# aicell-lab/bioengine-worker

Measured on AMD Instinct MI355X. Metric: cellpose_cyto3_512x512_imgs_per_sec, higher is better.
Workload: dtype bf16; 1 GPU; model=cellpose-cyto3 CPnet (nbase 2-32-64-128-256, style on, BN folded), global_batch=32, parallelism=dp1 (replica per GPU)

## Files before the change

### bioengine_worker_amd/ops/conv_pair.py

```python
from __future__ import annotations

from dataclasses import dataclass

import torch
import torch.nn.functional as F

from . import _native
from .conv import INMODES, PackedConv, _act_ref, _affine_stride, fused_conv2d, fused_conv2d_ref, out_hw

SUPPORTED = {
    (8, 32, "none", False, True, "none"),
    (32, 32, "none", False, False, "full"),
    (64, 32, "up2", True, False, "up2"),
    (32, 64, "pool2", False, False, "full"),
    (64, 64, "none", False, False, "full"),
    (128, 64, "up2", True, False, "up2"),
}
RESMODES = {"none": 0, "full": 1, "up2": 2}
FRAG_CONFIGS = {
    (64, 64, "none", False, False, "full"),
    (32, 64, "pool2", False, False, "full"),
    (128, 64, "up2", True, False, "up2"),
}
PROJ_CONFIGS = {
    (32, 64, "pool2", False, True, "none"),
}
SUPPORTED |= PROJ_CONFIGS


def pack_proj_frag(wp: torch.Tensor) -> torch.Tensor:
    cout, nchunk, kp = wp.shape
    assert cout == 64 and nchunk == 1 and kp == 32, "projection fragments: 32 -> 64 channels, 1x1"
    t = wp.reshape(4, 16, 4, 8)
    return t.permute(0, 2, 1, 3).contiguous().reshape(1, 4, 64, 8)


def unpack_proj_frag(wf: torch.Tensor) -> torch.Tensor:
    return wf.reshape(4, 4, 16, 8).permute(0, 2, 1, 3).contiguous().reshape(64, 1, 32)


def pack_frag(wp: torch.Tensor) -> torch.Tensor:
    cout, nchunk, kp = wp.shape
    assert cout == 64 and kp == 288, "fragment packing: 64 output channels, 3x3 taps of 32-channel chunks"
    t = wp.reshape(4, 16, nchunk, 9, 4, 8)
    return t.permute(2, 3, 0, 4, 1, 5).contiguous().reshape(nchunk, 9, 4, 64, 8)


def unpack_frag(wf: torch.Tensor) -> torch.Tensor:
    nchunk = wf.shape[0]
    t = wf.reshape(nchunk, 9, 4, 4, 16, 8)
    return t.permute(2, 4, 0, 1, 3, 5).contiguous().reshape(64, nchunk, 288)


@dataclass
class PairSpec:

    pa: PackedConv
    pb: PackedConv
    sa: torch.Tensor
    ta: torch.Tensor | None
    sb: torch.Tensor
    tb: torch.Tensor | None
    bias: torch.Tensor
    inmode: str = "none"
    pp: PackedConv | None = None
    sp: torch.Tensor | None = None
    tp: torch.Tensor | None = None
    frag_cache: dict | None = None
    bias_p: torch.Tensor | None = None
    proj_frag_cache: dict | None = None
    plain: "PairSpec | None" = None

    def proj_rounded(self, has_x2: bool, res: str) -> bool:
        return self.bias_p is not None and (self.cin, self.cm, self.inmode, has_x2, self.pp is not None, res) in PROJ_CONFIGS

    def frag_proj(self, device: torch.device) -> torch.Tensor:
        key = (str(device), self.pp.wp.data_ptr())
        if self.proj_frag_cache is None or self.proj_frag_cache.get("key") != key:
            self.proj_frag_cache = {"key": key, "w": pack_proj_frag(self.pp.wp.to(device))}
        return self.proj_frag_cache["w"]

    def frag(self, device: torch.device) -> tuple[torch.Tensor, torch.Tensor]:
        key = (str(device), self.pa.wp.data_ptr(), self.pb.wp.data_ptr())
        if self.frag_cache is None:
            self.frag_cache = {}
        if self.frag_cache.get("key") != key:
            self.frag_cache.update(key=key, w=(pack_frag(self.pa.wp.to(device)), pack_frag(self.pb.wp.to(device))))
        return self.frag_cache["w"]

    @property
    def cm(self) -> int:
        return self.pb.cout

    @property
    def cin(self) -> int:
        return self.pa.cin_pad

    def supports(self, has_x2: bool, res: str) -> bool:
        cfg = (self.cin, self.cm, self.inmode, has_x2, self.pp is not None, res)
        return cfg in SUPPORTED and (cfg in PROJ_CONFIGS) == (self.bias_p is not None)

    def without_proj(self) -> "PairSpec":
        if self.frag_cache is None:
            self.frag_cache = {}
        if self.plain is None:
            self.plain = PairSpec(pa=self.pa, pb=self.pb, sa=self.sa, ta=self.ta, sb=self.sb, tb=self.tb,
                                  bias=self.bias, inmode=self.inmode, frag_cache=self.frag_cache)
        return self.plain


def fold_bias(shift: torch.Tensor, scale: torch.Tensor, bias: torch.Tensor | None) -> torch.Tensor:
    if bias is None:
        return shift.clone()
    n = bias.numel()
    out = shift.clone()
    out[..., :n] = out[..., :n] + scale[:n] * bias.to(shift.device)
    return out


def conv_pair_ref(x, spec: PairSpec, *, ta=None, tb=None, x2=None, res=None, res_mode="none"):
    ta = spec.ta if ta is None else ta
    tb = spec.tb if tb is None else tb
    if spec.proj_rounded(x2 is not None, "none" if res is None else res_mode):
        proj = fused_conv2d_ref(x, spec.pp, scale=spec.sp, shift=spec.tp, inmode=spec.inmode)
        return conv_pair_ref(x, spec.without_proj(), ta=ta, tb=tb, res=proj, res_mode="full")
    xf = x.float()
    a = _act_ref(xf, None, spec.sa, ta, True, spec.inmode).to(torch.bfloat16).float()
    wa = spec.pa.w.to(a.device)
    if wa.shape[1] < a.shape[1]:
        wa = F.pad(wa, (0, 0, 0, 0, 0, a.shape[1] - wa.shape[1]))
    hA = F.conv2d(a, wa.to(torch.bfloat16).float(), None, padding=1)
    if x2 is not None:
        hA = hA + x2.float().permute(0, 3, 1, 2)
    C = hA.shape[1]
    sb = spec.sb[:C].view(1, C, 1, 1)
    tbv = tb.view(-1, tb.shape[-1], 1, 1)[:, :C] if tb.dim() == 2 else tb[:C].view(1, C, 1, 1)
    h = torch.relu(hA * sb + tbv).to(torch.bfloat16).float()
    y = F.conv2d(h, spec.pb.w.to(h.device).to(torch.bfloat16).float(), None, padding=1)
    if spec.pp is not None:
        p = _act_ref(xf, None, spec.sp, spec.tp, False, spec.inmode).to(torch.bfloat16).float()
        wp = spec.pp.w.to(p.device)
        if wp.shape[1] < p.shape[1]:
            wp = F.pad(wp, (0, 0, 0, 0, 0, p.shape[1] - wp.shape[1]))
        y = y + F.conv2d(p, wp.to(torch.bfloat16).float(), None)
    y = y + spec.bias.to(y.device).view(1, -1, 1, 1)
    y = y.permute(0, 2, 3, 1)
    if res is not None:
        r = res.float()
        if res_mode == "up2":
            r = r.repeat_interleave(2, 1).repeat_interleave(2, 2)
        y = y + r
    return y.to(x.dtype).contiguous()


def conv_pair(x: torch.Tensor, spec: PairSpec, *, ta=None, tb=None, x2=None, res=None, res_mode: str = "none",
              out: torch.Tensor | None = None) -> torch.Tensor:
    ta = spec.ta if ta is None else ta
    tb = spec.tb if tb is None else tb
    assert ta is not None and tb is not None, "conv_pair needs actA / actB shifts"
    if res is None:
        res_mode = "none"
    if not x.is_cuda:
        y = conv_pair_ref(x, spec, ta=ta, tb=tb, x2=x2, res=res, res_mode=res_mode)
        if out is not None:
            out.copy_(y)
            return out
        return y
    N, Hs, Ws, Cin = x.shape
    H, W = out_hw(x, spec.inmode)
    CM = spec.cm
    assert x.dtype == torch.bfloat16 and x.is_contiguous(), "conv_pair expects contiguous NHWC bf16"
    assert Cin == spec.cin, f"input channels {Cin} != packed {spec.cin}"
    if spec.proj_rounded(x2 is not None, res_mode):
        return _conv_pair_proj(x, spec, ta, tb, out)
    if not spec.supports(x2 is not None, res_mode):
        raise ValueError(f"conv_pair: unsupported configuration {(Cin, CM, spec.inmode, x2 is not None, spec.pp is not None, res_mode)}")
    if x2 is not None:
        assert x2.shape == (N, H, W, CM) and x2.dtype == torch.bfloat16 and x2.is_contiguous()
    if res_mode == "full":
        assert res.shape == (N, H, W, CM) and res.dtype == torch.bfloat16 and res.is_contiguous()
    elif res_mode == "up2":
        assert res.shape == (N, H // 2, W // 2, CM) and res.dtype == torch.bfloat16 and res.is_contiguous()
    if out is None:
        out = torch.empty(N, H, W, CM, device=x.device, dtype=torch.bfloat16)
    else:
        assert out.shape == (N, H, W, CM) and out.dtype == torch.bfloat16 and out.is_contiguous()
        assert out.data_ptr() != x.data_ptr(), "conv_pair cannot run in place"
    ta_ns = _affine_stride(ta, N, Cin)
    tb_ns = _affine_stride(tb, N, CM)
    pp = spec.pp
    waf = wbf = None
    if (Cin, CM, spec.inmode, x2 is not None, pp is not None, res_mode) in FRAG_CONFIGS:
        waf, wbf = spec.frag(x.device)
    _native.call(
        "be_conv_pair_frag",
        _native.ptr(x), _native.ptr(x2), _native.ptr(spec.sa), _native.ptr(ta), ta_ns, _native.ptr(spec.sb),
        _native.ptr(tb), tb_ns, _native.ptr(spec.sp), _native.ptr(spec.tp), _native.ptr(spec.pa.wp),
        _native.ptr(spec.pb.wp), _native.ptr(None if pp is None else pp.wp), _native.ptr(spec.bias),
        _native.ptr(res), _native.ptr(out), N, H, W, Hs, Ws, Cin, CM, INMODES[spec.inmode], int(pp is not None),
        RESMODES[res_mode], _native.ptr(waf), _native.ptr(wbf), _native.stream(x.device),
    )
    return out


def proj_fused(x: torch.Tensor, spec: PairSpec) -> bool:
    H, W = out_hw(x, spec.inmode)
    return x.is_cuda and bool(_native.hip().be_conv_pair_proj_takes(x.shape[0], H, W))


def _conv_pair_proj(x, spec: PairSpec, ta, tb, out):
    N, Hs, Ws, Cin = x.shape
    H, W = out_hw(x, spec.inmode)
    if not proj_fused(x, spec):
        proj = fused_conv2d(x, spec.pp, scale=spec.sp, shift=spec.tp, inmode=spec.inmode)
        return conv_pair(x, spec.without_proj(), ta=ta, tb=tb, res=proj, res_mode="full", out=out)
    CM = spec.cm
    if out is None:
        out = torch.empty(N, H, W, CM, device=x.device, dtype=torch.bfloat16)
    else:
        assert out.shape == (N, H, W, CM) and out.dtype == torch.bfloat16 and out.is_contiguous()
        assert out.data_ptr() != x.data_ptr(), "conv_pair cannot run in place"
    waf, wbf = spec.frag(x.device)
    _native.call(
        "be_conv_pair_proj",
        _native.ptr(x), _native.ptr(spec.sa), _native.ptr(ta), _affine_stride(ta, N, Cin), _native.ptr(spec.sb),
        _native.ptr(tb), _affine_stride(tb, N, CM), _native.ptr(spec.sp), _native.ptr(spec.tp), _native.ptr(spec.pa.wp),
        _native.ptr(spec.pb.wp), _native.ptr(spec.bias), _native.ptr(spec.bias_p), _native.ptr(out), N, H, W, Hs, Ws,
        Cin, CM, _native.ptr(waf), _native.ptr(wbf), _native.ptr(spec.frag_proj(x.device)), _native.stream(x.device),
    )
    return out


@dataclass
class HeadSpec:

    s: torch.Tensor
    t: torch.Tensor
    w: torch.Tensor
    b: torch.Tensor
    nh: int
    wh: torch.Tensor | None = None

    @staticmethod
    def k_order() -> list[int]:
        return [(kq * 4 + j) if j < 4 else (16 + kq * 4 + j - 4) for kq in range(4) for j in range(8)]

    @classmethod
    def build(cls, scale: torch.Tensor, shift: torch.Tensor, weight: torch.Tensor, bias: torch.Tensor | None):
        nh, cin = weight.shape[0], weight.shape[1]
        assert cin <= 32 and nh <= 16 and weight.shape[2:] == (1, 1)
        dev = weight.device
        w = torch.zeros(nh, 32, device=dev)
        w[:, :cin] = weight.detach().float().reshape(nh, cin)
        b = torch.zeros(16, device=dev)
        if bias is not None:
            b[:nh] = bias.detach().float()
        s = torch.zeros(32, device=dev)
        t = torch.zeros(32, device=dev)
        s[: scale.numel()] = scale.float()
        t[: shift.numel()] = shift.float()
        wp = torch.zeros(16, 32, device=dev)
        wp[:nh] = w[:, cls.k_order()]
        return cls(s=s.contiguous(), t=t.contiguous(), w=w, b=b.contiguous(), nh=nh,
                   wh=wp.to(torch.bfloat16).contiguous())


def head_ref(xout: torch.Tensor, head: HeadSpec) -> torch.Tensor:
    a = torch.relu(xout.float() * head.s.to(xout.device) + head.t.to(xout.device))
    w = head.w.to(a.device)
    if xout.dtype == torch.bfloat16:
        a = a.to(torch.bfloat16).float()
        w = w.to(torch.bfloat16).float()
    y = torch.einsum("nhwc,oc->nohw", a, w) + head.b[: head.nh].to(a.device).view(1, -1, 1, 1)
    return y.contiguous()


def conv_pair_head(x: torch.Tensor, spec: PairSpec, head: HeadSpec, *, ta=None, tb=None, res=None) -> torch.Tensor:
    ta = spec.ta if ta is None else ta
    tb = spec.tb if tb is None else tb
    assert ta is not None and tb is not None and res is not None
    if not x.is_cuda:
        return head_ref(conv_pair_ref(x, spec, ta=ta, tb=tb, res=res, res_mode="full"), head)
    N, H, W, Cin = x.shape
    assert spec.cin == 32 and spec.cm == 32 and spec.inmode == "none" and spec.pp is None, "head fusion: 32->32 only"
    assert x.dtype == torch.bfloat16 and x.is_contiguous() and Cin == 32
    assert res.shape == (N, H, W, 32) and res.dtype == torch.bfloat16 and res.is_contiguous()
    hout = torch.empty(N, head.nh, H, W, device=x.device, dtype=torch.float32)
    _native.call(
        "be_conv_pair_head",
        _native.ptr(x), _native.ptr(spec.sa), _native.ptr(ta), _affine_stride(ta, N, Cin), _native.ptr(spec.sb),
        _native.ptr(tb), _affine_stride(tb, N, 32), _native.ptr(spec.pa.wp), _native.ptr(spec.pb.wp),
        _native.ptr(spec.bias), _native.ptr(res), _native.ptr(head.s), _native.ptr(head.t), _native.ptr(head.wh),
        _native.ptr(head.b), _native.ptr(hout), head.nh, N, H, W, _native.stream(x.device),
    )
    return hout
```

### csrc/kernels/common.h

```cpp
#pragma once
#include <hip/hip_runtime.h>
#include <stdint.h>
#include <cstdio>
#include <cstdlib>

typedef uint16_t bf16_t;
typedef __attribute__((ext_vector_type(8))) short bf16x8;
typedef __attribute__((ext_vector_type(4))) float f32x4;
typedef __attribute__((ext_vector_type(4))) uint32_t u32x4;
typedef __attribute__((ext_vector_type(2))) uint32_t u32x2;

#define BE_WAVE 64

__device__ __forceinline__ float bf2f(uint16_t v) { return __uint_as_float(((uint32_t)v) << 16); }

typedef __attribute__((ext_vector_type(2))) float f32x2_t;
typedef __attribute__((ext_vector_type(2))) __bf16 bf16x2_t;

__device__ __forceinline__ uint16_t f2bf(float f) { return __builtin_bit_cast(uint16_t, (__bf16)f); }

__device__ __forceinline__ uint32_t pack2bf(float lo, float hi) {
  const f32x2_t v = {lo, hi};
  return __builtin_bit_cast(uint32_t, __builtin_convertvector(v, bf16x2_t));
}

typedef __attribute__((ext_vector_type(2))) short s16x2_t;
__device__ __forceinline__ uint32_t relu_bf16x2(uint32_t w) {
  const s16x2_t z = {0, 0};
  return __builtin_bit_cast(uint32_t, __builtin_elementwise_max(__builtin_bit_cast(s16x2_t, w), z));
}

__device__ __forceinline__ float lo_bf(uint32_t w) { return __uint_as_float(w << 16); }
__device__ __forceinline__ float hi_bf(uint32_t w) { return __uint_as_float(w & 0xffff0000u); }

__device__ __forceinline__ float wave_sum(float v) {
#pragma unroll
  for (int o = 32; o > 0; o >>= 1) v += __shfl_xor(v, o, 64);
  return v;
}
__device__ __forceinline__ float wave_max(float v) {
#pragma unroll
  for (int o = 32; o > 0; o >>= 1) v = fmaxf(v, __shfl_xor(v, o, 64));
  return v;
}

__device__ __forceinline__ int xcd_remap(int orig, int nwg) {
  const int q = nwg / 8, r = nwg % 8;
  const int xcd = orig % 8;
  const int base = (xcd < r) ? xcd * (q + 1) : r * (q + 1) + (xcd - r) * q;
  return base + orig / 8;
}

#define BE_CHECK_LAUNCH() ((int)hipGetLastError())

inline int be_env_int(const char* name, int dflt) {
  const char* e = getenv(name);
  return e ? atoi(e) : dflt;
}

#define BE_MAX_DEV 64
inline int be_cur_dev() {
  int d = 0;
  (void)hipGetDevice(&d);
  return (d < 0 || d >= BE_MAX_DEV) ? 0 : d;
}

inline const bf16_t* be_zero_page(int slot, size_t bytes) {
  static bf16_t* pages[4][BE_MAX_DEV] = {};
  bf16_t*& z = pages[slot & 3][be_cur_dev()];
  if (!z) {
    if (hipMalloc((void**)&z, bytes) != hipSuccess) { z = nullptr; return nullptr; }
    if (hipMemset(z, 0, bytes) != hipSuccess) return nullptr;
  }
  return z;
}
```

### csrc/kernels/conv_pair.hip

```cpp
#include <cstdlib>

#include "common.h"

namespace {

struct PairArgs {
  const bf16_t* x;
  const bf16_t* x2;
  const float* sa; const float* ta; int ta_ns;
  const float* sb; const float* tb; int tb_ns;
  const float* sp; const float* tp;
  const bf16_t* wa;
  const bf16_t* wb;
  const bf16_t* wp;
  const float* bias;
  const bf16_t* waf; const bf16_t* wbf;
  const bf16_t* wpf; const float* biasp;
  const bf16_t* res;
  bf16_t* out;
  const float* sh; const float* th;
  const bf16_t* wh;
  const float* bh;
  float* hout;
  int nh;
  int N, H, W, Hs, Ws, Cin;
  int tiles_x, tiles_y;
  unsigned long long* stamps;
};

namespace g32 {
constexpr int TW = 32, TH = 16, NW = 8;
#include "conv_pair_onegroup.inc"
}
using namespace g32;

unsigned long long* g_pair_stamps = nullptr;
int g_pair_stamps_cap = 0;

static int g_pair_var = (be_env_int("BE_PAIR_LATE_EPI", 1) ? 1 : 0) | (be_env_int("BE_PAIR_ROLL", 1) ? 2 : 0) |
                        (be_env_int("BE_PAIR_EARLY_AFF", 1) ? 4 : 0) | (be_env_int("BE_PAIR_EPIA", 0) ? 8 : 0) |
                        (be_env_int("BE_PAIR_SEPS", 0) ? 16 : 0) | (be_env_int("BE_PAIR_TOPEPI", 0) ? 32 : 0);

template <int CK, int CM, int INMODE, bool X2, bool PROJ, int RES, int NCA, bool HEAD, bool STAMP, int VAR>
int launch_pair_l(PairArgs a, int g, hipStream_t s) {
  using C = PC<CK, CM, INMODE, X2, PROJ, RES, NCA>;
  constexpr bool seps = (VAR & 16) != 0 && C::RESW && !HEAD;
  constexpr size_t lds = C::LDS + (seps ? (size_t)C::R_OUT * sizeof(bf16_t) : 0);
  static_assert(lds <= 160 * 1024, "LDS budget (separate output staging)");
  static bool attr_set[BE_MAX_DEV] = {};
  if (!attr_set[be_cur_dev()]) {
    hipFuncSetAttribute(
        reinterpret_cast<const void*>(&conv_pair_kernel<CK, CM, INMODE, X2, PROJ, RES, NCA, HEAD, STAMP, VAR>),
        hipFuncAttributeMaxDynamicSharedMemorySize, (int)lds);
    attr_set[be_cur_dev()] = true;
  }
  hipLaunchKernelGGL((conv_pair_kernel<CK, CM, INMODE, X2, PROJ, RES, NCA, HEAD, STAMP, VAR>), dim3(g), dim3(NT), lds, s,
                     a);
  return BE_CHECK_LAUNCH();
}

template <int CK, int CM, int INMODE, bool X2, bool PROJ, int RES, int NCA, bool HEAD = false, bool STAMP = false>
int launch_pair_k(PairArgs a, int g, hipStream_t s) {
  if constexpr (CM == 32 && CK == 32 && !HEAD) {
    if (g_pair_var & 16) {
      if constexpr (NCA == 1)
        if (g_pair_var & 32) return launch_pair_l<CK, CM, INMODE, X2, PROJ, RES, NCA, HEAD, STAMP, 48>(a, g, s);
      return launch_pair_l<CK, CM, INMODE, X2, PROJ, RES, NCA, HEAD, STAMP, 16>(a, g, s);
    }
  }
  if constexpr (CM == 32 && NCA == 1) {
    if (g_pair_var & 32) return launch_pair_l<CK, CM, INMODE, X2, PROJ, RES, NCA, HEAD, STAMP, 32>(a, g, s);
  }
  if constexpr (CM == 64 && RES != 0) {
    switch (g_pair_var & 15) {
      case 1: return launch_pair_l<CK, CM, INMODE, X2, PROJ, RES, NCA, HEAD, STAMP, 1>(a, g, s);
      case 2: return launch_pair_l<CK, CM, INMODE, X2, PROJ, RES, NCA, HEAD, STAMP, 2>(a, g, s);
      case 3: return launch_pair_l<CK, CM, INMODE, X2, PROJ, RES, NCA, HEAD, STAMP, 3>(a, g, s);
      case 5: return launch_pair_l<CK, CM, INMODE, X2, PROJ, RES, NCA, HEAD, STAMP, 5>(a, g, s);
      case 7: return launch_pair_l<CK, CM, INMODE, X2, PROJ, RES, NCA, HEAD, STAMP, 7>(a, g, s);
      case 15: return launch_pair_l<CK, CM, INMODE, X2, PROJ, RES, NCA, HEAD, STAMP, 15>(a, g, s);
      default: break;
    }
  }
  return launch_pair_l<CK, CM, INMODE, X2, PROJ, RES, NCA, HEAD, STAMP, 0>(a, g, s);
}

template <int CK, int CM, int INMODE, bool X2, bool PROJ, int RES, int NCA, bool HEAD = false>
int launch_pair(PairArgs a, int grid_cap, hipStream_t s) {
  a.tiles_x = (a.W + TW - 1) / TW;
  a.tiles_y = (a.H + TH - 1) / TH;
  const int tiles = a.N * a.tiles_x * a.tiles_y;
  int g = grid_cap > 0 ? grid_cap : 256;
  if (g > tiles) g = tiles;
  if (g < 1) return 0;
  a.stamps = nullptr;
  if constexpr (!HEAD && !PROJ && CK == 32) {
    if (g_pair_stamps != nullptr) {
      if (g > g_pair_stamps_cap) return -30;
      a.stamps = g_pair_stamps;
      return launch_pair_k<CK, CM, INMODE, X2, PROJ, RES, NCA, HEAD, true>(a, g, s);
    }
  }
  return launch_pair_k<CK, CM, INMODE, X2, PROJ, RES, NCA, HEAD, false>(a, g, s);
}

#ifndef PP_VAR
#define PP_VAR 1
#endif
#ifndef PP_GW
#define PP_GW 4
#endif
namespace ppk {
constexpr int GW = PP_GW, GT = GW * 64;
constexpr int NTP = 2 * GT;
constexpr int RPW = TH / GW;
constexpr int IN_B = IPIX * 64;
constexpr int H_B = RPIX * 64;
constexpr int OUTW_B = RPW * TW * 64;
constexpr int RB = IN_B;
constexpr int WSTR = 9 * 32 + 16;
constexpr int W_B = 32 * WSTR * 2;
constexpr int APT = 40 / GW, BPT = 32 / GW;
constexpr int TLAST0 = GW * (APT - 1);
constexpr int HU = IPIX * 4;
constexpr int HUPT = (HU + GT - 1) / GT;
static_assert(H_B <= RB && GW * OUTW_B <= RB, "ping-pong region overlays");
static_assert(APT * GW >= RPT && (APT - 1) * GW <= 2 * RH && BPT * GW * 16 == TH * TW, "tile maps");
static_assert(GW == 4 || GW == 8, "group size");
}

struct PPHalo {
  u32x4 h[ppk::HUPT];
  float4 aff[4];
};

__device__ __forceinline__ int pp_in_off(int pi, int c) {
  const int y = pi / IW, x = pi - y * IW;
  return pi * 64 + ((c ^ ((((x >> 2) ^ y) & 1) << 1)) << 4);
}

template <int INMODE, int CIN, bool INT = false>
__device__ __forceinline__ void pp_issue_halo(const PairArgs& a, TileXY t, int ch, int gt, PPHalo& hr) {
  const int c = ch * 32 + (gt & 3) * 8;
  hr.aff[0] = *reinterpret_cast<const float4*>(a.sa + c);
  hr.aff[1] = *reinterpret_cast<const float4*>(a.sa + c + 4);
  const float* tr = a.ta + (size_t)t.n * a.ta_ns + c;
  hr.aff[2] = *reinterpret_cast<const float4*>(tr);
  hr.aff[3] = *reinterpret_cast<const float4*>(tr + 4);
#pragma unroll
  for (int i = 0; i < ppk::HUPT; ++i) {
    const int pi = min(gt + i * ppk::GT, ppk::HU - 1) >> 2;
    const int y = pi / IW, x = pi - y * IW;
    const int gy = INT ? t.ty0 - 2 + y : min(max(t.ty0 - 2 + y, 0), a.H - 1);
    const int gx = INT ? t.tx0 - 2 + x : min(max(t.tx0 - 2 + x, 0), a.W - 1);
    if constexpr (INMODE == 0)
      hr.h[i] = *reinterpret_cast<const u32x4*>(a.x + (((size_t)t.n * a.Hs + gy) * a.Ws + gx) * CIN + c);
    else
      hr.h[i] = *reinterpret_cast<const u32x4*>(a.x + (((size_t)t.n * a.Hs + (gy >> 1)) * a.Ws + (gx >> 1)) * CIN + c);
  }
}

__device__ __forceinline__ bool pp_interior(const PairArgs& a, TileXY t) {
  return t.ty0 >= 2 && t.ty0 + TH + 2 <= a.H && t.tx0 >= 2 && t.tx0 + TW + 2 <= a.W;
}

template <bool INT>
__device__ __forceinline__ void pp_commit(const PairArgs& a, TileXY t, int gt, const PPHalo& hr, unsigned char* rin) {
  float sc[8], sh[8];
  unpack_aff(hr.aff, sc, sh);
  const int c = gt & 3;
#pragma unroll
  for (int i = 0; i < ppk::HUPT; ++i) {
    const int u = gt + i * ppk::GT;
    if (u >= ppk::HU) continue;
    const int pi = u >> 2;
    const int y = pi / IW, x = pi - y * IW;
    const int gy = t.ty0 - 2 + y, gx = t.tx0 - 2 + x;
    u32x4 pk = (u32x4){0u, 0u, 0u, 0u};
    if (INT || (gy >= 0 && gy < a.H && gx >= 0 && gx < a.W)) {
#pragma unroll
      for (int j = 0; j < 4; ++j)
        pk[j] = relu_bf16x2(pack2bf(fmaf(lo_bf(hr.h[i][j]), sc[2 * j], sh[2 * j]),
                                    fmaf(hi_bf(hr.h[i][j]), sc[2 * j + 1], sh[2 * j + 1])));
    }
    *reinterpret_cast<u32x4*>(rin + pi * 64 + ((c ^ ((((x >> 2) ^ y) & 1) << 1)) << 4)) = pk;
  }
}

__device__ __forceinline__ void pp_mma_a(f32x4 (&acc)[2][ppk::APT], const unsigned char* rin, const bf16_t* wa, int gw,
                                         int lrow, int kq) {
  const int par = (gw >> 1) & 1;
  const int b0 = ((gw >> 1) * IW + (gw & 1) * 16 + lrow) * 64;
  int A0[3][2];
#pragma unroll
  for (int dx = 0; dx < 3; ++dx)
#pragma unroll
    for (int pr = 0; pr < 2; ++pr)
      A0[dx][pr] = b0 + dx * 64 + ((kq ^ (((((lrow + dx) >> 2) ^ par ^ pr) & 1) << 1)) << 4);
  int L[3][2];
  const int tl = gw + ppk::TLAST0;
  if (tl < 2 * RH) {
    const int ryl = tl >> 1, rxl = (tl & 1) * 16 + lrow;
#pragma unroll
    for (int dx = 0; dx < 3; ++dx)
#pragma unroll
      for (int pr = 0; pr < 2; ++pr)
        L[dx][pr] = (ryl * IW + rxl + dx) * 64 + ((kq ^ (((((lrow + dx) >> 2) ^ ryl ^ pr) & 1) << 1)) << 4);
  } else {
    int ry9 = (tl - 2 * RH) * 8 + (lrow >> 1), rx9 = 32 + (lrow & 1);
    if (ry9 >= RH) { ry9 = 0; rx9 = 0; }
#pragma unroll
    for (int dx = 0; dx < 3; ++dx)
#pragma unroll
      for (int pr = 0; pr < 2; ++pr)
        L[dx][pr] = (ry9 * IW + rx9 + dx) * 64 + ((kq ^ ((((ry9 & 1) ^ pr) & 1) << 1)) << 4);
  }
  auto frags = [&](int ks, bf16x8 (&af)[2], bf16x8 (&bf)[ppk::APT]) {
    const int dy = ks / 3, dx = ks % 3;
#pragma unroll
    for (int ct = 0; ct < 2; ++ct)
      af[ct] = *reinterpret_cast<const bf16x8*>(wa + (ct * 16 + lrow) * ppk::WSTR + ks * 32 + kq * 8);
#pragma unroll
    for (int j = 0; j < ppk::APT - 1; ++j)
      bf[j] = *reinterpret_cast<const bf16x8*>(rin + A0[dx][dy & 1] + j * (ppk::GW / 2) * IW * 64 + dy * IW * 64);
    bf[ppk::APT - 1] = *reinterpret_cast<const bf16x8*>(rin + L[dx][dy & 1] + dy * IW * 64);
  };
  bf16x8 af[2], afn[2], bf[ppk::APT];
  frags(0, af, bf);
#pragma unroll
  for (int ks = 0; ks < 9; ++ks) {
    const bool more = ks + 1 < 9;
    const int kn = more ? ks + 1 : ks, dy = kn / 3, dx = kn % 3;
#pragma unroll
    for (int j = 0; j < ppk::APT; ++j) {
#pragma unroll
      for (int ct = 0; ct < 2; ++ct) {
        acc[ct][j] = __builtin_amdgcn_mfma_f32_16x16x32_bf16(af[ct], bf[j], acc[ct][j], 0, 0, 0);
        if (j == 0 && more)
          afn[ct] = *reinterpret_cast<const bf16x8*>(wa + (ct * 16 + lrow) * ppk::WSTR + kn * 32 + kq * 8);
      }
      if (more) {
        if (j < ppk::APT - 1)
          bf[j] = *reinterpret_cast<const bf16x8*>(rin + A0[dx][dy & 1] + j * (ppk::GW / 2) * IW * 64 + dy * IW * 64);
        else
          bf[j] = *reinterpret_cast<const bf16x8*>(rin + L[dx][dy & 1] + dy * IW * 64);
      }
      __builtin_amdgcn_sched_barrier(0);
    }
    if (more) {
      af[0] = afn[0];
      af[1] = afn[1];
    }
  }
}

struct PPSkip {
  u32x2 xv[ppk::APT][2];
};

__device__ __forceinline__ bool pp_last(int gw, int lrow, int& ry, int& rx) {
  const int tl = gw + ppk::TLAST0;
  if (tl < 2 * RH) {
    ry = tl >> 1;
    rx = (tl & 1) * 16 + lrow;
    return true;
  }
  ry = (tl - 2 * RH) * 8 + (lrow >> 1);
  rx = 32 + (lrow & 1);
  return ry < RH;
}

__device__ __forceinline__ void pp_issue_skip(const PairArgs& a, TileXY t, int gw, int lrow, int kq, PPSkip& sk) {
#pragma unroll
  for (int j = 0; j < ppk::APT; ++j) {
    int ry, rx;
    if (j < ppk::APT - 1) {
      ry = (gw >> 1) + (ppk::GW / 2) * j;
      rx = (gw & 1) * 16 + lrow;
    } else {
      pp_last(gw, lrow, ry, rx);
    }
    const int gy = min(max(t.ty0 - 1 + ry, 0), a.H - 1), gx = min(max(t.tx0 - 1 + rx, 0), a.W - 1);
    const bf16_t* xp = a.x2 + (((size_t)t.n * a.H + gy) * a.W + gx) * 32 + kq * 4;
#pragma unroll
    for (int ct = 0; ct < 2; ++ct) sk.xv[j][ct] = *reinterpret_cast<const u32x2*>(xp + ct * 16);
  }
}

template <bool X2, bool INT>
__device__ __forceinline__ void pp_epi_a(const PairArgs& a, TileXY t, const f32x4 (&acc)[2][ppk::APT],
                                         unsigned char* rh, const float4 (&s)[2], const float4 (&sh)[2],
                                         const PPSkip& sk, int gw, int lrow, int kq) {
#pragma unroll
  for (int ct = 0; ct < 2; ++ct) {
    const int hc = ((2 * ct) | (kq >> 1));
    const int hw = (((gw >> 1) * RW + (gw & 1) * 16 + lrow) * 64) + ((hc ^ ((lrow >> 1) & 3)) << 4) + (kq & 1) * 8;
#pragma unroll
    for (int j = 0; j < ppk::APT; ++j) {
      int ry, rx, off;
      if (j < ppk::APT - 1) {
        ry = (gw >> 1) + (ppk::GW / 2) * j;
        rx = (gw & 1) * 16 + lrow;
        off = hw + j * (ppk::GW / 2) * RW * 64;
      } else {
        if (!pp_last(gw, lrow, ry, rx)) continue;
        off = (ry * RW + rx) * 64 + ((hc ^ ((rx >> 1) & 3)) << 4) + (kq & 1) * 8;
      }
      const int gy = t.ty0 - 1 + ry, gx = t.tx0 - 1 + rx;
      float v0 = acc[ct][j][0], v1 = acc[ct][j][1], v2 = acc[ct][j][2], v3 = acc[ct][j][3];
      if constexpr (X2) {
        u32x2 xv = sk.xv[j][ct];
        asm volatile("" : "+v"(xv));
        v0 += lo_bf(xv[0]); v1 += hi_bf(xv[0]); v2 += lo_bf(xv[1]); v3 += hi_bf(xv[1]);
      }
      u32x2 st = (u32x2){0u, 0u};
      if (INT || (gy >= 0 && gy < a.H && gx >= 0 && gx < a.W)) {
        st[0] = relu_bf16x2(pack2bf(fmaf(v0, s[ct].x, sh[ct].x), fmaf(v1, s[ct].y, sh[ct].y)));
        st[1] = relu_bf16x2(pack2bf(fmaf(v2, s[ct].z, sh[ct].z), fmaf(v3, s[ct].w, sh[ct].w)));
      }
      *reinterpret_cast<u32x2*>(rh + off) = st;
    }
  }
}

__device__ __forceinline__ void pp_mma_b(f32x4 (&acc)[2][ppk::BPT], const unsigned char* rh, const bf16_t* wb, int gw,
                                         int lrow, int kq) {
  int B0[3];
#pragma unroll
  for (int dx = 0; dx < 3; ++dx) B0[dx] = ((ppk::RPW * gw) * RW + lrow + dx) * 64 + ((kq ^ (((lrow + dx) >> 1) & 3)) << 4);
  auto frags = [&](int ks, bf16x8 (&af)[2], bf16x8 (&bf)[ppk::BPT]) {
    const int dy = ks / 3, dx = ks % 3;
#pragma unroll
    for (int ct = 0; ct < 2; ++ct)
      af[ct] = *reinterpret_cast<const bf16x8*>(wb + (ct * 16 + lrow) * ppk::WSTR + ks * 32 + kq * 8);
#pragma unroll
    for (int pt = 0; pt < ppk::BPT; ++pt)
      bf[pt] = *reinterpret_cast<const bf16x8*>(rh + B0[dx] + ((pt >> 1) + dy) * RW * 64 + (pt & 1) * 16 * 64);
  };
  bf16x8 af[2], afn[2], bf[ppk::BPT];
  frags(0, af, bf);
#pragma unroll
  for (int ks = 0; ks < 9; ++ks) {
    const bool more = ks + 1 < 9;
    const int kn = more ? ks + 1 : ks, dy = kn / 3, dx = kn % 3;
#pragma unroll
    for (int pt = 0; pt < ppk::BPT; ++pt) {
#pragma unroll
      for (int ct = 0; ct < 2; ++ct) {
        acc[ct][pt] = __builtin_amdgcn_mfma_f32_16x16x32_bf16(af[ct], bf[pt], acc[ct][pt], 0, 0, 0);
        if (pt == 0 && more)
          afn[ct] = *reinterpret_cast<const bf16x8*>(wb + (ct * 16 + lrow) * ppk::WSTR + kn * 32 + kq * 8);
      }
      if (more) bf[pt] = *reinterpret_cast<const bf16x8*>(rh + B0[dx] + ((pt >> 1) + dy) * RW * 64 + (pt & 1) * 16 * 64);
      __builtin_amdgcn_sched_barrier(0);
    }
    if (more) {
      af[0] = afn[0];
      af[1] = afn[1];
    }
  }
}

struct PPRes {
  u32x2 rv[ppk::BPT][2];
  float4 bias[2];
};

template <int RES>
__device__ __forceinline__ void pp_issue_res(const PairArgs& a, TileXY t, int gw, int lrow, int kq, PPRes& r) {
#pragma unroll
  for (int pt = 0; pt < ppk::BPT; ++pt) {
    if constexpr (RES == 0) {
      r.rv[pt][0] = r.rv[pt][1] = (u32x2){0u, 0u};
      continue;
    }
    const int py = min(t.ty0 + ppk::RPW * gw + (pt >> 1), a.H - 1), px = min(t.tx0 + (pt & 1) * 16 + lrow, a.W - 1);
    const bf16_t* rp = RES == 1 ? a.res + (((size_t)t.n * a.H + py) * a.W + px) * 32 + kq * 4
                                : a.res + (((size_t)t.n * (a.H >> 1) + (py >> 1)) * (a.W >> 1) + (px >> 1)) * 32 + kq * 4;
#pragma unroll
    for (int ct = 0; ct < 2; ++ct) r.rv[pt][ct] = *reinterpret_cast<const u32x2*>(rp + ct * 16);
  }
#pragma unroll
  for (int ct = 0; ct < 2; ++ct) r.bias[ct] = *reinterpret_cast<const float4*>(a.bias + ct * 16 + kq * 4);
}

template <int RES>
__device__ __forceinline__ void pp_epi_b(const PairArgs& a, TileXY t, const f32x4 (&acc)[2][ppk::BPT], const PPRes& r,
                                         unsigned char* ws, int gw, int lrow, int kq, bool act) {
  const __amdgpu_buffer_rsrc_t rs = __builtin_amdgcn_make_buffer_rsrc(
      a.out + (size_t)t.n * a.H * a.W * 32, (short)0, a.H * a.W * 64, 0x00020000);
  if constexpr (PP_VAR & 16) {
#pragma unroll
    for (int pt = 0; pt < ppk::BPT; ++pt) {
      const int py = t.ty0 + ppk::RPW * gw + (pt >> 1), px = t.tx0 + (pt & 1) * 16 + lrow;
      const bool ok = act && py < a.H && px < a.W;
#pragma unroll
      for (int ct = 0; ct < 2; ++ct) {
        u32x2 rv = r.rv[pt][ct];
        asm volatile("" : "+v"(rv));
        u32x2 st;
        st[0] = pack2bf(acc[ct][pt][0] + r.bias[ct].x + lo_bf(rv[0]), acc[ct][pt][1] + r.bias[ct].y + hi_bf(rv[0]));
        st[1] = pack2bf(acc[ct][pt][2] + r.bias[ct].z + lo_bf(rv[1]), acc[ct][pt][3] + r.bias[ct].w + hi_bf(rv[1]));
        const int off = ok ? ((py * a.W + px) * 32 + ct * 16 + kq * 4) * 2 : 0x7ffffff0;
        __builtin_amdgcn_raw_buffer_store_b64(st, rs, off, 0, 0);
      }
    }
    return;
  }
#pragma unroll
  for (int ct = 0; ct < 2; ++ct) {
    const int ow = lrow * 64 + ((((2 * ct) | (kq >> 1)) ^ ((lrow >> 1) & 3)) << 4) + (kq & 1) * 8;
#pragma unroll
    for (int pt = 0; pt < ppk::BPT; ++pt) {
      u32x2 rv = r.rv[pt][ct];
      if constexpr (RES != 0) asm volatile("" : "+v"(rv));
      u32x2 st;
      st[0] = pack2bf(acc[ct][pt][0] + r.bias[ct].x + lo_bf(rv[0]), acc[ct][pt][1] + r.bias[ct].y + hi_bf(rv[0]));
      st[1] = pack2bf(acc[ct][pt][2] + r.bias[ct].z + lo_bf(rv[1]), acc[ct][pt][3] + r.bias[ct].w + hi_bf(rv[1]));
      *reinterpret_cast<u32x2*>(ws + ow + ((pt >> 1) * 32 + (pt & 1) * 16) * 64) = st;
    }
  }
  __builtin_amdgcn_fence(__ATOMIC_RELEASE, "wavefront");
  __builtin_amdgcn_wave_barrier();
  __builtin_amdgcn_fence(__ATOMIC_ACQUIRE, "wavefront");
  const int lane = lrow + 16 * kq;
  const int rd = (lane >> 2) * 64 + (((lane & 3) ^ ((lane >> 3) & 3)) << 4);
  const int py0 = t.ty0 + ppk::RPW * gw, px0 = t.tx0 + (lane >> 2);
#pragma unroll
  for (int it = 0; it < 2 * ppk::RPW; ++it) {
    const int py = py0 + (it >> 1), px = px0 + (it & 1) * 16;
    const u32x4 v = *reinterpret_cast<const u32x4*>(ws + rd + it * 1024);
    const int off = (act && py < a.H && px < a.W) ? ((py * a.W + px) * 32 + (lane & 3) * 8) * 2 : 0x7ffffff0;
    __builtin_amdgcn_raw_buffer_store_b128(v, rs, off, 0, 0);
    __builtin_amdgcn_sched_barrier(0);
  }
}

__device__ __forceinline__ void pp_epi_head(const PairArgs& a, TileXY t, const f32x4 (&acc)[2][ppk::BPT], const PPRes& r,
                                            const HeadRegs& hr, int gw, int lrow, int kq, bool act) {
  const f32x4 zero = {0.f, 0.f, 0.f, 0.f};
  const __amdgpu_buffer_rsrc_t rs = __builtin_amdgcn_make_buffer_rsrc(
      a.hout + (size_t)t.n * a.nh * a.H * a.W, (short)0, a.nh * a.H * a.W * 4, 0x00020000);
#pragma unroll
  for (int pt = 0; pt < ppk::BPT; ++pt) {
    u32x4 bw;
#pragma unroll
    for (int ct = 0; ct < 2; ++ct) {
      u32x2 rv = r.rv[pt][ct];
      asm volatile("" : "+v"(rv));
      const float4 bias = r.bias[ct];
      const uint32_t o0 = pack2bf(acc[ct][pt][0] + bias.x + lo_bf(rv[0]), acc[ct][pt][1] + bias.y + hi_bf(rv[0]));
      const uint32_t o1 = pack2bf(acc[ct][pt][2] + bias.z + lo_bf(rv[1]), acc[ct][pt][3] + bias.w + hi_bf(rv[1]));
      bw[2 * ct] = relu_bf16x2(pack2bf(fmaf(lo_bf(o0), hr.s[ct].x, hr.t[ct].x), fmaf(hi_bf(o0), hr.s[ct].y, hr.t[ct].y)));
      bw[2 * ct + 1] = relu_bf16x2(pack2bf(fmaf(lo_bf(o1), hr.s[ct].z, hr.t[ct].z), fmaf(hi_bf(o1), hr.s[ct].w, hr.t[ct].w)));
    }
    const f32x4 y = __builtin_amdgcn_mfma_f32_16x16x32_bf16(hr.w, *reinterpret_cast<const bf16x8*>(&bw), zero, 0, 0, 0);
    const int py = t.ty0 + ppk::RPW * gw + (pt >> 1), px = t.tx0 + (pt & 1) * 16 + lrow;
    const bool ok = act && py < a.H && px < a.W;
    const float bb[4] = {hr.b.x, hr.b.y, hr.b.z, hr.b.w};
#pragma unroll
    for (int i = 0; i < 4; ++i) {
      const int co = kq * 4 + i;
      const int off = (ok && co < a.nh) ? ((co * a.H + py) * a.W + px) * 4 : 0x7ffffff0;
      __builtin_amdgcn_raw_buffer_store_b32(__float_as_uint(y[i] + bb[i]), rs, off, 0, 0);
    }
  }
}

namespace pps {
constexpr int PST = 24;
constexpr int PSP = 8;
constexpr int KPA = 96, WSTRA = KPA + 16;
constexpr int WSTRP = 48;
constexpr int IN_B = IPIX * PST * 2;
constexpr int P_B = TH * TW * PSP * 2;
constexpr int R_B = ppk::H_B > IN_B ? ppk::H_B : IN_B;
constexpr int RB = R_B + P_B;
constexpr int WA_B = 32 * WSTRA * 2, WB_B = 32 * ppk::WSTR * 2, WP_B = 32 * WSTRP * 2;
constexpr int LDS = 2 * RB + WA_B + WB_B + WP_B;
constexpr int HUPT = (IPIX + ppk::GT - 1) / ppk::GT;
static_assert(LDS <= 128 * 1024 && ppk::GW * ppk::OUTW_B <= R_B, "stem ping-pong LDS budget");
}

struct PPHalo8 {
  u32x4 h[pps::HUPT];
  float4 aff[4], paff[4];
};

template <bool INT = false>
__device__ __forceinline__ void pp8_issue_halo(const PairArgs& a, TileXY t, int gt, PPHalo8& hr) {
  hr.aff[0] = *reinterpret_cast<const float4*>(a.sa);
  hr.aff[1] = *reinterpret_cast<const float4*>(a.sa + 4);
  const float* tr = a.ta + (size_t)t.n * a.ta_ns;
  hr.aff[2] = *reinterpret_cast<const float4*>(tr);
  hr.aff[3] = *reinterpret_cast<const float4*>(tr + 4);
  hr.paff[0] = *reinterpret_cast<const float4*>(a.sp);
  hr.paff[1] = *reinterpret_cast<const float4*>(a.sp + 4);
  hr.paff[2] = *reinterpret_cast<const float4*>(a.tp);
  hr.paff[3] = *reinterpret_cast<const float4*>(a.tp + 4);
#pragma unroll
  for (int i = 0; i < pps::HUPT; ++i) {
    const int pi = min(gt + i * ppk::GT, IPIX - 1);
    const int y = pi / IW, x = pi - y * IW;
    const int gy = INT ? t.ty0 - 2 + y : min(max(t.ty0 - 2 + y, 0), a.H - 1);
    const int gx = INT ? t.tx0 - 2 + x : min(max(t.tx0 - 2 + x, 0), a.W - 1);
    hr.h[i] = *reinterpret_cast<const u32x4*>(a.x + (((size_t)t.n * a.Hs + gy) * a.Ws + gx) * 8);
  }
}

template <bool INT>
__device__ __forceinline__ void pp8_commit(const PairArgs& a, TileXY t, int gt, const PPHalo8& hr, unsigned char* rin,
                                           unsigned char* preg) {
  float sc[8], sh[8], ps[8], pt[8];
  unpack_aff(hr.aff, sc, sh);
  unpack_aff(hr.paff, ps, pt);
#pragma unroll
  for (int i = 0; i < pps::HUPT; ++i) {
    const int pi = gt + i * ppk::GT;
    if (pi >= IPIX) continue;
    const int iy = pi / IW, ix = pi - iy * IW;
    const int gy = t.ty0 - 2 + iy, gx = t.tx0 - 2 + ix;
    const bool in = INT || (gy >= 0 && gy < a.H && gx >= 0 && gx < a.W);
    float v[8];
#pragma unroll
    for (int j = 0; j < 4; ++j) { v[2 * j] = lo_bf(hr.h[i][j]); v[2 * j + 1] = hi_bf(hr.h[i][j]); }
    u32x4 pk = (u32x4){0u, 0u, 0u, 0u};
    if (in) {
#pragma unroll
      for (int j = 0; j < 4; ++j)
        pk[j] = relu_bf16x2(pack2bf(fmaf(v[2 * j], sc[2 * j], sh[2 * j]), fmaf(v[2 * j + 1], sc[2 * j + 1], sh[2 * j + 1])));
    }
    *reinterpret_cast<u32x4*>(rin + pi * pps::PST * 2) = pk;
    if (iy >= 2 && iy < TH + 2 && ix >= 2 && ix < TW + 2) {
      u32x4 pp = (u32x4){0u, 0u, 0u, 0u};
      if (in) {
#pragma unroll
        for (int j = 0; j < 4; ++j)
          pp[j] = pack2bf(fmaf(v[2 * j], ps[2 * j], pt[2 * j]), fmaf(v[2 * j + 1], ps[2 * j + 1], pt[2 * j + 1]));
      }
      *reinterpret_cast<u32x4*>(preg + ((iy - 2) * TW + (ix - 2)) * pps::PSP * 2) = pp;
    }
  }
}

__device__ __forceinline__ void pp8_mma_a(f32x4 (&acc)[2][ppk::APT], const unsigned char* rin, const bf16_t* wa, int gw,
                                          int lrow, int kq) {
  int toff[3];
#pragma unroll
  for (int ks = 0; ks < 3; ++ks) {
    int tap = ks * 4 + kq;
    if (tap >= 9) tap = 0;
    toff[ks] = ((tap / 3) * IW + tap % 3) * pps::PST * 2;
  }
  const int b0 = ((gw >> 1) * IW + (gw & 1) * 16 + lrow) * pps::PST * 2;
  int ryl, rxl;
  if (!pp_last(gw, lrow, ryl, rxl)) { ryl = 0; rxl = 0; }
  const int bl = (ryl * IW + rxl) * pps::PST * 2;
#pragma unroll
  for (int ks = 0; ks < 3; ++ks) {
    bf16x8 af[2], bf[ppk::APT];
#pragma unroll
    for (int ct = 0; ct < 2; ++ct)
      af[ct] = *reinterpret_cast<const bf16x8*>(wa + (ct * 16 + lrow) * pps::WSTRA + ks * 32 + kq * 8);
#pragma unroll
    for (int j = 0; j < ppk::APT - 1; ++j)
      bf[j] = *reinterpret_cast<const bf16x8*>(rin + b0 + toff[ks] + j * (ppk::GW / 2) * IW * pps::PST * 2);
    bf[ppk::APT - 1] = *reinterpret_cast<const bf16x8*>(rin + bl + toff[ks]);
#pragma unroll
    for (int ct = 0; ct < 2; ++ct)
#pragma unroll
      for (int j = 0; j < ppk::APT; ++j)
        acc[ct][j] = __builtin_amdgcn_mfma_f32_16x16x32_bf16(af[ct], bf[j], acc[ct][j], 0, 0, 0);
  }
}

__device__ __forceinline__ void pp8_mma_p(f32x4 (&acc)[2][ppk::BPT], const unsigned char* preg, const bf16_t* wp, int gw,
                                          int lrow, int kq) {
  bf16x8 af[2], bf[ppk::BPT];
#pragma unroll
  for (int ct = 0; ct < 2; ++ct) af[ct] = *reinterpret_cast<const bf16x8*>(wp + (ct * 16 + lrow) * pps::WSTRP + kq * 8);
#pragma unroll
  for (int pt = 0; pt < ppk::BPT; ++pt) {
    const int oy = ppk::RPW * gw + (pt >> 1), ox = (pt & 1) * 16 + lrow;
    bf[pt] = *reinterpret_cast<const bf16x8*>(preg + (oy * TW + ox) * pps::PSP * 2);
  }
#pragma unroll
  for (int ct = 0; ct < 2; ++ct)
#pragma unroll
    for (int pt = 0; pt < ppk::BPT; ++pt)
      acc[ct][pt] = __builtin_amdgcn_mfma_f32_16x16x32_bf16(af[ct], bf[pt], acc[ct][pt], 0, 0, 0);
}

template <bool STEM> struct PPHaloOf { using T = PPHalo; };
template <> struct PPHaloOf<true> { using T = PPHalo8; };

template <int NCA, int INMODE, bool X2, int RES, bool HEAD, bool STEM = false, bool STAMP = false>
__global__ __launch_bounds__(ppk::NTP, ppk::GW == 4 ? 2 : 4) void conv_pair_pp_kernel(PairArgs a) {
  static_assert(!STEM || (NCA == 1 && INMODE == 0 && !X2 && RES == 0 && !HEAD), "stem configuration");
  constexpr int CIN = 32 * NCA;
  constexpr int RB = STEM ? pps::RB : ppk::RB;
  unsigned long long ph_work[7] = {0, 0, 0, 0, 0, 0, 0}, ph_wait[7] = {0, 0, 0, 0, 0, 0, 0};
  unsigned long long tstamp = STAMP ? __builtin_amdgcn_s_memtime() : 0;
  auto pre = [&](int i) {
    if constexpr (STAMP) {
      const unsigned long long tn = __builtin_amdgcn_s_memtime();
      ph_work[i] += tn - tstamp;
      tstamp = tn;
    }
  };
  auto post = [&](int i) {
    if constexpr (STAMP) {
      const unsigned long long tn = __builtin_amdgcn_s_memtime();
      ph_wait[i] += tn - tstamp;
      tstamp = tn;
    }
  };
  constexpr int NST = HEAD ? 4 * ppk::BPT : ((PP_VAR & 16) ? 2 * ppk::BPT : 2 * ppk::RPW);
  extern __shared__ __attribute__((aligned(16))) unsigned char smem[];
  const int tid0 = threadIdx.x;
  const int total = a.N * a.tiles_x * a.tiles_y;
  const int t0 = (int)(((long long)blockIdx.x * total) / gridDim.x);
  const int t1 = (int)(((long long)(blockIdx.x + 1) * total) / gridDim.x);
  if (t0 >= t1) return;
  bf16_t* wl = reinterpret_cast<bf16_t*>(smem + 2 * RB);
  const bf16_t* wb = wl + (STEM ? 32 * pps::WSTRA : NCA * 32 * ppk::WSTR);
  const bf16_t* wp = wb + 32 * ppk::WSTR;
  if constexpr (STEM) {
    for (int u = tid0; u < 32 * (12 + 36 + 4); u += ppk::NTP) {
      const int r = u / 52, q = u % 52;
      const bf16_t* src;
      bf16_t* dst;
      if (q < 12) { src = a.wa + (size_t)r * 96 + q * 8; dst = wl + r * pps::WSTRA + q * 8; }
      else if (q < 48) { src = a.wb + (size_t)r * 288 + (q - 12) * 8; dst = const_cast<bf16_t*>(wb) + r * ppk::WSTR + (q - 12) * 8; }
      else { src = a.wp + (size_t)r * 32 + (q - 48) * 8; dst = const_cast<bf16_t*>(wp) + r * pps::WSTRP + (q - 48) * 8; }
      *reinterpret_cast<u32x4*>(dst) = *reinterpret_cast<const u32x4*>(src);
    }
  } else {
    for (int u = tid0; u < (NCA + 1) * 32 * 36; u += ppk::NTP) {
      const int pnl = u / (32 * 36), q = u % (32 * 36), r = q / 36, k8 = q % 36;
      const bf16_t* src = pnl < NCA ? a.wa + ((size_t)r * NCA + pnl) * 288 + k8 * 8 : a.wb + (size_t)r * 288 + k8 * 8;
      *reinterpret_cast<u32x4*>(wl + pnl * 32 * ppk::WSTR + r * ppk::WSTR + k8 * 8) = *reinterpret_cast<const u32x4*>(src);
    }
  }
  const int grp = __builtin_amdgcn_readfirstlane(tid0 / ppk::GT);
  const int gt0 = tid0 & (ppk::GT - 1);
  unsigned char* reg = smem + grp * RB;
  HeadRegs hr;
  if constexpr (HEAD) load_head(a, tid0 & 15, (tid0 & 63) >> 4, hr);
  typename PPHaloOf<STEM>::T halo;
  auto issue0 = [&](TileXY nx, int gtv) {
    if constexpr (STEM) {
      if (pp_interior(a, nx)) pp8_issue_halo<true>(a, nx, gtv, halo);
      else pp8_issue_halo<false>(a, nx, gtv, halo);
    } else {
      if (pp_interior(a, nx)) pp_issue_halo<INMODE, CIN, true>(a, nx, 0, gtv, halo);
      else pp_issue_halo<INMODE, CIN>(a, nx, 0, gtv, halo);
    }
  };
  if constexpr (STEM) pp8_issue_halo<false>(a, tile_xy(a, min(t0 + grp, t1 - 1)), gt0, halo);
  else pp_issue_halo<INMODE, CIN>(a, tile_xy(a, min(t0 + grp, t1 - 1)), 0, gt0, halo);
  __builtin_amdgcn_s_waitcnt((0x7 << 4) | (0xf << 8));
  __syncthreads();
  if (grp == 1) __builtin_amdgcn_s_barrier();
  const int iters = (t1 - t0 + 1) >> 1;
  for (int k = 0; k < iters; ++k) {
    int gt = gt0;
    asm volatile("" : "+v"(gt));
    const int gw = __builtin_amdgcn_readfirstlane(gt >> 6), lane = gt & 63, lrow = lane & 15, kq = lane >> 4;
    const int t = t0 + 2 * k + grp;
    const bool act = t < t1;
    const TileXY cur = tile_xy(a, act ? t : t1 - 1);
    const bool inner = pp_interior(a, cur);
    f32x4 acc_a[2][ppk::APT];
    float4 sb[2], tb[2];
    PPSkip sk;
#pragma unroll
    for (int c = 0; c < NCA; ++c) {
      constexpr int NW = (PP_VAR & 2) ? 0 : NST;
      if (c == 0) __builtin_amdgcn_s_waitcnt((NW & 0xf) | (0x7 << 4) | (0xf << 8) | ((NW >> 4) << 14));
      int gc = gt0;
      asm volatile("" : "+v"(gc));
      if constexpr (STEM) {
        if (inner) pp8_commit<true>(a, cur, gc, halo, reg, reg + pps::R_B);
        else pp8_commit<false>(a, cur, gc, halo, reg, reg + pps::R_B);
      } else {
        if (inner) pp_commit<true>(a, cur, gc, halo, reg);
        else pp_commit<false>(a, cur, gc, halo, reg);
      }
      pre(2 * c);
      __syncthreads();
      post(2 * c);
      if constexpr (!STEM) {
        if (c + 1 < NCA) {
          if (inner) pp_issue_halo<INMODE, CIN, true>(a, cur, c + 1, gt, halo);
          else pp_issue_halo<INMODE, CIN>(a, cur, c + 1, gt, halo);
        }
      }
      if (c == NCA - 1) {
#pragma unroll
        for (int ct = 0; ct < 2; ++ct) {
          sb[ct] = *reinterpret_cast<const float4*>(a.sb + ct * 16 + kq * 4);
          tb[ct] = *reinterpret_cast<const float4*>(a.tb + (size_t)cur.n * a.tb_ns + ct * 16 + kq * 4);
        }
        if constexpr (X2) pp_issue_skip(a, cur, gw, lrow, kq, sk);
      }
      if (c == 0) {
#pragma unroll
        for (int i = 0; i < 2; ++i)
#pragma unroll
          for (int j = 0; j < ppk::APT; ++j) acc_a[i][j] = (f32x4){0.f, 0.f, 0.f, 0.f};
      }
      if constexpr (!(PP_VAR & 4)) __builtin_amdgcn_s_setprio(1);
      if constexpr (STEM) pp8_mma_a(acc_a, reg, wl, gw, lrow, kq);
      else pp_mma_a(acc_a, reg, wl + c * 32 * ppk::WSTR, gw, lrow, kq);
      if constexpr (!(PP_VAR & 4)) __builtin_amdgcn_s_setprio(0);
      pre(2 * c + 1);
      __syncthreads();
      post(2 * c + 1);
    }
    int g3 = gt0;
    asm volatile("" : "+v"(g3));
    if (inner) pp_epi_a<X2, true>(a, cur, acc_a, reg, sb, tb, sk, gw, g3 & 15, (g3 & 63) >> 4);
    else pp_epi_a<X2, false>(a, cur, acc_a, reg, sb, tb, sk, gw, g3 & 15, (g3 & 63) >> 4);
    PPRes res;
    if constexpr (PP_VAR & 1) pp_issue_res<RES>(a, cur, gw, g3 & 15, (g3 & 63) >> 4, res);
    if constexpr (PP_VAR & 8) issue0(tile_xy(a, min(t + 2, t1 - 1)), g3);
    pre(2 * NCA);
    __syncthreads();
    post(2 * NCA);
    int g4 = gt0;
    asm volatile("" : "+v"(g4));
    const int lrow4 = g4 & 15, kq4 = (g4 & 63) >> 4;
    f32x4 acc_b[2][ppk::BPT];
    if constexpr (!(PP_VAR & 1)) pp_issue_res<RES>(a, cur, gw, lrow4, kq4, res);
#pragma unroll
    for (int i = 0; i < 2; ++i)
#pragma unroll
      for (int j = 0; j < ppk::BPT; ++j) acc_b[i][j] = (f32x4){0.f, 0.f, 0.f, 0.f};
    if constexpr (!(PP_VAR & 4)) __builtin_amdgcn_s_setprio(1);
    pp_mma_b(acc_b, reg, wb, gw, lrow4, kq4);
    if constexpr (STEM) pp8_mma_p(acc_b, reg + pps::R_B, wp, gw, lrow4, kq4);
    if constexpr (!(PP_VAR & 4)) __builtin_amdgcn_s_setprio(0);
    pre(2 * NCA + 1);
    __syncthreads();
    post(2 * NCA + 1);
    int g5 = gt0;
    asm volatile("" : "+v"(g5));
    const int lrow5 = g5 & 15, kq5 = (g5 & 63) >> 4;
    auto next_halo = [&]() { issue0(tile_xy(a, min(t + 2, t1 - 1)), g5); };
    if constexpr (!(PP_VAR & 10)) next_halo();
    __builtin_amdgcn_sched_barrier(0);
    if constexpr (HEAD) pp_epi_head(a, cur, acc_b, res, hr, gw, lrow5, kq5, act);
    else pp_epi_b<RES>(a, cur, acc_b, res, reg + gw * ppk::OUTW_B, gw, lrow5, kq5, act);
    if constexpr (PP_VAR & 2) next_halo();
    pre(2 * NCA + 2);
    __syncthreads();
    post(2 * NCA + 2);
  }
  if (grp == 0) __builtin_amdgcn_s_barrier();
  if constexpr (STAMP) {
    if ((tid0 & (ppk::GT - 1)) < 16) {
      const int k = tid0 & 15;
      unsigned long long v = 0;
#pragma unroll
      for (int i = 0; i < 7; ++i) {
        if (k == i) v = ph_work[i];
        if (k == 8 + i) v = ph_wait[i];
      }
      if (k == 15) v = (unsigned long long)iters;
      a.stamps[((size_t)blockIdx.x * 2 + grp) * 16 + k] = v;
    }
  }
}

unsigned long long* g_pp_stamps = nullptr;
int g_pp_stamps_cap = 0;

template <int NCA, int INMODE, bool X2, int RES, bool HEAD, bool STEM = false>
int launch_pair_pp(PairArgs a, int grid_cap, hipStream_t s) {
  constexpr int lds = STEM ? pps::LDS : 2 * ppk::RB + (NCA + 1) * ppk::W_B;
  static_assert(lds <= 160 * 1024, "ping-pong LDS budget");
  a.tiles_x = (a.W + TW - 1) / TW;
  a.tiles_y = (a.H + TH - 1) / TH;
  const int tiles = a.N * a.tiles_x * a.tiles_y;
  int g = grid_cap > 0 ? grid_cap : 256;
  if (g > tiles) g = tiles;
  if (g < 1) return 0;
  a.stamps = nullptr;
  static bool attr_set[BE_MAX_DEV] = {};
  if (!attr_set[be_cur_dev()]) {
    hipFuncSetAttribute(reinterpret_cast<const void*>(&conv_pair_pp_kernel<NCA, INMODE, X2, RES, HEAD, STEM>),
                        hipFuncAttributeMaxDynamicSharedMemorySize, lds);
    attr_set[be_cur_dev()] = true;
  }
  if (g_pp_stamps != nullptr) {
    if (g > g_pp_stamps_cap) return -30;
    a.stamps = g_pp_stamps;
    static bool attr_st[BE_MAX_DEV] = {};
    if (!attr_st[be_cur_dev()]) {
      hipFuncSetAttribute(reinterpret_cast<const void*>(&conv_pair_pp_kernel<NCA, INMODE, X2, RES, HEAD, STEM, true>),
                          hipFuncAttributeMaxDynamicSharedMemorySize, lds);
      attr_st[be_cur_dev()] = true;
    }
    hipLaunchKernelGGL((conv_pair_pp_kernel<NCA, INMODE, X2, RES, HEAD, STEM, true>), dim3(g), dim3(ppk::NTP), lds, s, a);
    return BE_CHECK_LAUNCH();
  }
  hipLaunchKernelGGL((conv_pair_pp_kernel<NCA, INMODE, X2, RES, HEAD, STEM>), dim3(g), dim3(ppk::NTP), lds, s, a);
  return BE_CHECK_LAUNCH();
}

#include "conv_pair_pp64.inc"

template <int NCA, int INMODE, bool X2, int RES, bool PROJ = false>
int launch_pair_pp64(PairArgs a, int grid_cap, hipStream_t s) {
  constexpr int lds = PROJ ? pp64::LDS_PROJ : pp64::LDS;
  a.tiles_x = (a.W + pp64::TS - 1) / pp64::TS;
  a.tiles_y = (a.H + pp64::TS - 1) / pp64::TS;
  const int tiles = a.N * a.tiles_x * a.tiles_y;
  int g = grid_cap > 0 ? grid_cap : 256;
  if (g > tiles) g = tiles;
  if (g < 1) return 0;
  a.stamps = nullptr;
  static bool attr_set[BE_MAX_DEV] = {};
  if (!attr_set[be_cur_dev()]) {
    (void)hipFuncSetAttribute(reinterpret_cast<const void*>(&pp64::conv_pair_pp64_kernel<NCA, INMODE, X2, RES, false, PROJ>),
                              hipFuncAttributeMaxDynamicSharedMemorySize, lds);
    (void)hipFuncSetAttribute(reinterpret_cast<const void*>(&pp64::conv_pair_pp64_kernel<NCA, INMODE, X2, RES, true, PROJ>),
                              hipFuncAttributeMaxDynamicSharedMemorySize, lds);
    attr_set[be_cur_dev()] = true;
  }
  if (g_pp_stamps != nullptr) {
    if (g > g_pp_stamps_cap) return -30;
    a.stamps = g_pp_stamps;
    hipLaunchKernelGGL((pp64::conv_pair_pp64_kernel<NCA, INMODE, X2, RES, true, PROJ>), dim3(g), dim3(pp64::NTP), lds, s, a);
    return BE_CHECK_LAUNCH();
  }
  hipLaunchKernelGGL((pp64::conv_pair_pp64_kernel<NCA, INMODE, X2, RES, false, PROJ>), dim3(g), dim3(pp64::NTP), lds, s, a);
  return BE_CHECK_LAUNCH();
}
}

static int g_pair_grid = be_env_int("BE_PAIR_GRID", 0);

static int g_pair_pp = be_env_int("BE_PAIR_PP", 1);

static int g_pair_pp_stem = be_env_int("BE_PAIR_PP_STEM", 1);

static bool pp_ok(const PairArgs& a, int grid_cap) {
  if (!g_pair_pp || g_pair_stamps != nullptr) return false;
  const long long tiles = (long long)a.N * ((a.W + TW - 1) / TW) * ((a.H + TH - 1) / TH);
  const int g = grid_cap > 0 ? grid_cap : 256;
  return tiles >= 2LL * g;
}

static int g_pair_pp64 = be_env_int("BE_PAIR_PP64", 1);

static bool pp64_size_ok(int N, int H, int W, int grid_cap) {
  if (!g_pair_pp64 || g_pair_stamps != nullptr) return false;
  const long long tiles = (long long)N * ((W + pp64::TS - 1) / pp64::TS) * ((H + pp64::TS - 1) / pp64::TS);
  const int g = grid_cap > 0 ? grid_cap : 256;
  return tiles >= 2LL * g;
}

static bool pp64_ok(const PairArgs& a, int grid_cap) { return a.waf && a.wbf && pp64_size_ok(a.N, a.H, a.W, grid_cap); }

static int g_pair_pp64_proj = be_env_int("BE_PAIR_PP64_PROJ", 1);

extern "C" {

int be_conv_pair_pp64_takes(int N, int H, int W) { return pp64_size_ok(N, H, W, g_pair_grid) ? 1 : 0; }

int be_conv_pair_proj_takes(int N, int H, int W) { return g_pair_pp64_proj && be_conv_pair_pp64_takes(N, H, W); }

int be_conv_pair_set_proj_fusion(int on) {
  g_pair_pp64_proj = on;
  return 0;
}

int be_conv_pair_set_grid(int blocks) {
  g_pair_grid = blocks;
  return 0;
}

int be_conv_pair_set_stamps(void* buf, int cap_workgroups) {
  g_pair_stamps = static_cast<unsigned long long*>(buf);
  g_pair_stamps_cap = buf ? cap_workgroups : 0;
  return 0;
}

int be_conv_pair_pp_set_stamps(void* buf, int cap_workgroups) {
  g_pp_stamps = static_cast<unsigned long long*>(buf);
  g_pp_stamps_cap = buf ? cap_workgroups : 0;
  return 0;
}

int be_conv_pair_lds(int cin, int cm, int inmode, int x2, int proj, int res) {
  (void)inmode; (void)x2; (void)res;
  if (cm == 32 && cin == 8 && proj) return (int)PC<8, 32, 0, false, true, 0, 1>::LDS;
  if (cm == 32 && cin == 32) return (int)PC<32, 32, 0, false, false, 1, 1>::LDS;
  if (cm == 32 && cin == 64) return (int)PC<32, 32, 1, true, false, 2, 2>::LDS;
  if (cm == 64) return (int)PC<32, 64, 0, false, false, 1, 2>::LDS;
  return -1;
}

int be_conv_pair_frag(const void* x, const void* x2, const float* sa, const float* ta, int ta_ns, const float* sb,
                      const float* tb, int tb_ns, const float* sp, const float* tp, const void* wa, const void* wb,
                      const void* wp, const float* bias, const void* res, void* out, int N, int H, int W, int Hs,
                      int Ws, int Cin, int CM, int inmode, int proj, int resmode, const void* waf, const void* wbf,
                      hipStream_t stream) {
  PairArgs a;
  a.waf = (const bf16_t*)waf; a.wbf = (const bf16_t*)wbf; a.wpf = nullptr; a.biasp = nullptr;
  a.x = (const bf16_t*)x; a.x2 = (const bf16_t*)x2;
  a.sa = sa; a.ta = ta; a.ta_ns = ta_ns; a.sb = sb; a.tb = tb; a.tb_ns = tb_ns; a.sp = sp; a.tp = tp;
  a.wa = (const bf16_t*)wa; a.wb = (const bf16_t*)wb; a.wp = (const bf16_t*)wp; a.bias = bias;
  a.res = (const bf16_t*)res; a.out = (bf16_t*)out;
  a.N = N; a.H = H; a.W = W; a.Hs = Hs; a.Ws = Ws; a.Cin = Cin;
  a.sh = a.th = a.bh = nullptr; a.wh = nullptr; a.hout = nullptr; a.nh = 0;
  const bool hx2 = x2 != nullptr;
  if (!sa || !ta || !sb || !tb || !wa || !wb || !bias || !out || !x) return -20;
  if ((resmode != 0) != (res != nullptr)) return -21;
  if (proj && (!sp || !tp || !wp)) return -22;
  const int g = g_pair_grid;
  if (CM == 32 && Cin == 8 && inmode == 0 && !hx2 && proj && resmode == 0) {
    if (g_pair_pp_stem && pp_ok(a, g) && Hs == H && Ws == W)
      return launch_pair_pp<1, 0, false, 0, false, true>(a, g, stream);
    return launch_pair<8, 32, 0, false, true, 0, 1>(a, g, stream);
  }
  if (CM == 32 && Cin == 32 && inmode == 0 && !hx2 && !proj && resmode == 1) {
    if (pp_ok(a, g) && Hs == H && Ws == W) return launch_pair_pp<1, 0, false, 1, false>(a, g, stream);
    return launch_pair<32, 32, 0, false, false, 1, 1>(a, g, stream);
  }
  if (CM == 32 && Cin == 64 && inmode == 1 && hx2 && !proj && resmode == 2) {
    if (pp_ok(a, g) && 2 * Hs == H && 2 * Ws == W)
      return launch_pair_pp<2, 1, true, 2, false>(a, g, stream);
    return launch_pair<32, 32, 1, true, false, 2, 2>(a, g, stream);
  }
  if (CM == 64 && Cin == 32 && inmode == 2 && !hx2 && !proj && resmode == 1) {
    if (pp64_ok(a, g) && Hs == 2 * H && Ws == 2 * W) return launch_pair_pp64<1, 2, false, 1>(a, g, stream);
    return launch_pair<32, 64, 2, false, false, 1, 1>(a, g, stream);
  }
  if (CM == 64 && Cin == 64 && inmode == 0 && !hx2 && !proj && resmode == 1) {
    if (pp64_ok(a, g) && Hs == H && Ws == W) return launch_pair_pp64<2, 0, false, 1>(a, g, stream);
    return launch_pair<32, 64, 0, false, false, 1, 2>(a, g, stream);
  }
  if (CM == 64 && Cin == 128 && inmode == 1 && hx2 && !proj && resmode == 2) {
    if (pp64_ok(a, g) && 2 * Hs == H && 2 * Ws == W) return launch_pair_pp64<4, 1, true, 2>(a, g, stream);
    return launch_pair<32, 64, 1, true, false, 2, 4>(a, g, stream);
  }
  return -23;
}

int be_conv_pair_proj(const void* x, const float* sa, const float* ta, int ta_ns, const float* sb, const float* tb,
                      int tb_ns, const float* sp, const float* tp, const void* wa, const void* wb, const float* bias,
                      const float* biasp, void* out, int N, int H, int W, int Hs, int Ws, int Cin, int CM,
                      const void* waf, const void* wbf, const void* wpf, hipStream_t stream) {
  if (!x || !sa || !ta || !sb || !tb || !wa || !wb || !bias || !out) return -20;
  if (!sp || !tp || !wpf || !biasp || !waf || !wbf) return -22;
  if (CM != 64 || Cin != 32 || Hs != 2 * H || Ws != 2 * W) return -23;
  if (!be_conv_pair_proj_takes(N, H, W)) return -25;
  PairArgs a;
  a.waf = (const bf16_t*)waf; a.wbf = (const bf16_t*)wbf; a.wpf = (const bf16_t*)wpf; a.biasp = biasp;
  a.x = (const bf16_t*)x; a.x2 = nullptr;
  a.sa = sa; a.ta = ta; a.ta_ns = ta_ns; a.sb = sb; a.tb = tb; a.tb_ns = tb_ns; a.sp = sp; a.tp = tp;
  a.wa = (const bf16_t*)wa; a.wb = (const bf16_t*)wb; a.wp = nullptr; a.bias = bias;
  a.res = nullptr; a.out = (bf16_t*)out;
  a.N = N; a.H = H; a.W = W; a.Hs = Hs; a.Ws = Ws; a.Cin = Cin;
  a.sh = a.th = a.bh = nullptr; a.wh = nullptr; a.hout = nullptr; a.nh = 0;
  return launch_pair_pp64<1, 2, false, 0, true>(a, g_pair_grid, stream);
}

int be_conv_pair(const void* x, const void* x2, const float* sa, const float* ta, int ta_ns, const float* sb,
                 const float* tb, int tb_ns, const float* sp, const float* tp, const void* wa, const void* wb,
                 const void* wp, const float* bias, const void* res, void* out, int N, int H, int W, int Hs, int Ws,
                 int Cin, int CM, int inmode, int proj, int resmode, hipStream_t stream) {
  return be_conv_pair_frag(x, x2, sa, ta, ta_ns, sb, tb, tb_ns, sp, tp, wa, wb, wp, bias, res, out, N, H, W, Hs, Ws, Cin,
                           CM, inmode, proj, resmode, nullptr, nullptr, stream);
}

int be_conv_pair_head(const void* x, const float* sa, const float* ta, int ta_ns, const float* sb, const float* tb,
                      int tb_ns, const void* wa, const void* wb, const float* bias, const void* res, const float* sh,
                      const float* th, const void* wh, const float* bh, float* hout, int nh, int N, int H, int W,
                      hipStream_t stream) {
  if (!x || !sa || !ta || !sb || !tb || !wa || !wb || !bias || !res || !sh || !th || !wh || !bh || !hout) return -20;
  if (nh < 1 || nh > 16) return -24;
  PairArgs a;
  a.x = (const bf16_t*)x; a.x2 = nullptr;
  a.sa = sa; a.ta = ta; a.ta_ns = ta_ns; a.sb = sb; a.tb = tb; a.tb_ns = tb_ns; a.sp = nullptr; a.tp = nullptr;
  a.wa = (const bf16_t*)wa; a.wb = (const bf16_t*)wb; a.wp = nullptr; a.bias = bias;
  a.res = (const bf16_t*)res; a.out = nullptr; a.waf = a.wbf = nullptr; a.wpf = nullptr; a.biasp = nullptr;
  a.sh = sh; a.th = th; a.wh = (const bf16_t*)wh; a.bh = bh; a.hout = hout; a.nh = nh;
  a.N = N; a.H = H; a.W = W; a.Hs = H; a.Ws = W; a.Cin = 32;
  if (pp_ok(a, g_pair_grid)) return launch_pair_pp<1, 0, false, 1, true>(a, g_pair_grid, stream);
  return launch_pair<32, 32, 0, false, false, 1, 1, true>(a, g_pair_grid, stream);
}

}
```

### csrc/kernels/conv_pair_pp64.inc

```
namespace pp64 {
constexpr int TS = 16;
constexpr int GW = 4, GT = GW * 64, NTP = 2 * GT;
constexpr int RW = TS + 2, RPIX = RW * RW;
constexpr int IW = TS + 4, IPIX = IW * IW;
constexpr int IN_B = IPIX * 64;
constexpr int H_B = RPIX * 128;
constexpr int OUTW_B = 8 * TS * 64;
constexpr int RB = H_B;
constexpr int LDS = 2 * RB;
constexpr int APT = 11, BPT = 8;
constexpr int HU = IPIX * 4, HUPT = (HU + GT - 1) / GT;
constexpr int WD = 3;
constexpr int WSTEP = 4 * 64 * 8;
constexpr int P_B = TS * TS * 64;
constexpr int LDS_PROJ = 2 * (RB + P_B);
static_assert(IN_B <= RB && GW * OUTW_B <= RB, "region overlays");
static_assert(LDS_PROJ <= 128 * 1024, "LDS budget of the ping-pong kernels");

__device__ __forceinline__ TileXY tile16(const PairArgs& a, int t) {
  const int tpi = a.tiles_x * a.tiles_y;
  TileXY r;
  r.n = t / tpi;
  const int q = t - r.n * tpi;
  r.ty0 = (q / a.tiles_x) * TS;
  r.tx0 = (q % a.tiles_x) * TS;
  return r;
}

__device__ __forceinline__ bool interior(const PairArgs& a, TileXY t) {
  return t.ty0 >= 2 && t.ty0 + TS + 2 <= a.H && t.tx0 >= 2 && t.tx0 + TS + 2 <= a.W;
}

template <int INMODE>
struct Halo {
  u32x4 h[HUPT][INMODE == 2 ? 4 : 1];
  float4 aff[4];
};

template <int CIN, int INMODE>
__device__ __forceinline__ void issue_halo(const PairArgs& a, TileXY t, int ch, int gt, Halo<INMODE>& hr) {
  const int c = ch * 32 + (gt & 3) * 8;
  if (ch == 0) {
    hr.aff[0] = *reinterpret_cast<const float4*>(a.sa + c);
    hr.aff[1] = *reinterpret_cast<const float4*>(a.sa + c + 4);
    const float* tr = a.ta + (size_t)t.n * a.ta_ns + c;
    hr.aff[2] = *reinterpret_cast<const float4*>(tr);
    hr.aff[3] = *reinterpret_cast<const float4*>(tr + 4);
  }
#pragma unroll
  for (int i = 0; i < HUPT; ++i) {
    const int pi = min(gt + i * GT, HU - 1) >> 2;
    const int y = pi / IW, x = pi - y * IW;
    const int gy = min(max(t.ty0 - 2 + y, 0), a.H - 1);
    const int gx = min(max(t.tx0 - 2 + x, 0), a.W - 1);
    if constexpr (INMODE == 0) {
      hr.h[i][0] = *reinterpret_cast<const u32x4*>(a.x + (((size_t)t.n * a.Hs + gy) * a.Ws + gx) * CIN + c);
    } else if constexpr (INMODE == 1) {
      hr.h[i][0] = *reinterpret_cast<const u32x4*>(a.x + (((size_t)t.n * a.Hs + (gy >> 1)) * a.Ws + (gx >> 1)) * CIN + c);
    } else {
      const bf16_t* base = a.x + (((size_t)t.n * a.Hs + 2 * gy) * a.Ws + 2 * gx) * CIN + c;
      hr.h[i][0] = *reinterpret_cast<const u32x4*>(base);
      hr.h[i][1] = *reinterpret_cast<const u32x4*>(base + CIN);
      hr.h[i][2] = *reinterpret_cast<const u32x4*>(base + (size_t)a.Ws * CIN);
      hr.h[i][3] = *reinterpret_cast<const u32x4*>(base + (size_t)a.Ws * CIN + CIN);
    }
  }
}

struct PAff {
  float4 f[4];
};

__device__ __forceinline__ void issue_paff(const PairArgs& a, int gt, PAff& p) {
  const int c = (gt & 3) * 8;
  p.f[0] = *reinterpret_cast<const float4*>(a.sp + c);
  p.f[1] = *reinterpret_cast<const float4*>(a.sp + c + 4);
  p.f[2] = *reinterpret_cast<const float4*>(a.tp + c);
  p.f[3] = *reinterpret_cast<const float4*>(a.tp + c + 4);
}

__device__ __forceinline__ int p_off(int oy, int ox, int c) {
  return (oy * TS + ox) * 64 + ((c ^ ((((ox >> 2) ^ oy) & 1) << 1)) << 4);
}

template <int INMODE, bool PROJ = false>
__device__ __forceinline__ void commit(const PairArgs& a, TileXY t, int ch, int gt, bool inner, const Halo<INMODE>& hr,
                                       unsigned char* rin, const PAff* paff = nullptr, unsigned char* preg = nullptr) {
  const int c = gt & 3, cc = ch * 32 + c * 8;
  float sc[8], sh[8];
  float ps[8], pt[8];
  if constexpr (PROJ) unpack_aff(paff->f, ps, pt);
  if (ch == 0) {
    unpack_aff(hr.aff, sc, sh);
  } else {
    float4 f[4];
    f[0] = *reinterpret_cast<const float4*>(a.sa + cc);
    f[1] = *reinterpret_cast<const float4*>(a.sa + cc + 4);
    const float* tr = a.ta + (size_t)t.n * a.ta_ns + cc;
    f[2] = *reinterpret_cast<const float4*>(tr);
    f[3] = *reinterpret_cast<const float4*>(tr + 4);
    unpack_aff(f, sc, sh);
  }
#pragma unroll
  for (int i = 0; i < HUPT; ++i) {
    const int u = gt + i * GT;
    if (u >= HU) continue;
    const int pi = u >> 2;
    const int y = pi / IW, x = pi - y * IW;
    const int gy = t.ty0 - 2 + y, gx = t.tx0 - 2 + x;
    u32x4 pk = (u32x4){0u, 0u, 0u, 0u}, pp = (u32x4){0u, 0u, 0u, 0u};
    if (inner || (gy >= 0 && gy < a.H && gx >= 0 && gx < a.W)) {
#pragma unroll
      for (int j = 0; j < 4; ++j) {
        float lo = lo_bf(hr.h[i][0][j]), hi = hi_bf(hr.h[i][0][j]);
        if constexpr (INMODE == 2) {
          lo = fmaxf(fmaxf(lo, lo_bf(hr.h[i][1][j])), fmaxf(lo_bf(hr.h[i][2][j]), lo_bf(hr.h[i][3][j])));
          hi = fmaxf(fmaxf(hi, hi_bf(hr.h[i][1][j])), fmaxf(hi_bf(hr.h[i][2][j]), hi_bf(hr.h[i][3][j])));
        }
        pk[j] = relu_bf16x2(pack2bf(fmaf(lo, sc[2 * j], sh[2 * j]), fmaf(hi, sc[2 * j + 1], sh[2 * j + 1])));
        if constexpr (PROJ) pp[j] = pack2bf(fmaf(lo, ps[2 * j], pt[2 * j]), fmaf(hi, ps[2 * j + 1], pt[2 * j + 1]));
      }
    }
    *reinterpret_cast<u32x4*>(rin + pi * 64 + ((c ^ ((((x >> 2) ^ y) & 1) << 1)) << 4)) = pk;
    if constexpr (PROJ) {
      if (y >= 2 && y < TS + 2 && x >= 2 && x < TS + 2) *reinterpret_cast<u32x4*>(preg + p_off(y - 2, x - 2, c)) = pp;
    }
  }
}

__device__ __forceinline__ bool a_pix(int ph, int j, int lrow, int& ry, int& rx) {
  if (j < 9) {
    ry = 9 * ph + j;
    rx = lrow;
    return true;
  }
  if (j == 9) {
    ry = 8 * ph + (lrow >> 1);
    rx = 16 + (lrow & 1);
    return true;
  }
  ry = 16 + (lrow >> 1);
  rx = 16 + (lrow & 1);
  const bool ok = ph == 0 && ry < RW;
  if (!ok) { ry = 0; rx = 0; }
  return ok;
}

struct WPre {
  bf16x8 w[WD][2];
};

__device__ __forceinline__ const bf16_t* w_lane(const bf16_t* wf, int cp, int lane) {
  return wf + cp * 2 * 512 + lane * 8;
}

__device__ __forceinline__ void issue_w(const bf16_t* wl, WPre& p) {
#pragma unroll
  for (int d = 0; d < WD; ++d)
#pragma unroll
    for (int ct = 0; ct < 2; ++ct) p.w[d][ct] = *reinterpret_cast<const bf16x8*>(wl + d * WSTEP + ct * 512);
}

template <int NS, int NPT, typename RD>
__device__ __forceinline__ void mma_run(f32x4 (&acc)[2][NPT], const unsigned char* reg, const bf16_t* wl, const WPre& pre,
                                        RD rd) {
  bf16x8 w[NS][2];
#pragma unroll
  for (int d = 0; d < WD; ++d) {
    w[d][0] = pre.w[d][0];
    w[d][1] = pre.w[d][1];
  }
  bf16x8 bf[NPT];
#pragma unroll
  for (int j = 0; j < NPT; ++j) bf[j] = *reinterpret_cast<const bf16x8*>(reg + rd(0, j));
#pragma unroll
  for (int s = 0; s < NS; ++s) {
    if (s + WD < NS) {
#pragma unroll
      for (int ct = 0; ct < 2; ++ct)
        w[s + WD][ct] = *reinterpret_cast<const bf16x8*>(wl + (s + WD) * WSTEP + ct * 512);
    }
    __builtin_amdgcn_sched_barrier(0);
#pragma unroll
    for (int j = 0; j < NPT; ++j) {
#pragma unroll
      for (int ct = 0; ct < 2; ++ct)
        acc[ct][j] = __builtin_amdgcn_mfma_f32_16x16x32_bf16(w[s][ct], bf[j], acc[ct][j], 0, 0, 0);
      if (s + 1 < NS) bf[j] = *reinterpret_cast<const bf16x8*>(reg + rd(s + 1, j));
      __builtin_amdgcn_sched_barrier(0);
    }
  }
}

__device__ __forceinline__ void mma_a(f32x4 (&acc)[2][APT], const unsigned char* rin, const bf16_t* wl, const WPre& pre,
                                      int ph, int lrow, int kq) {
  int A0[3];
#pragma unroll
  for (int dx = 0; dx < 3; ++dx)
    A0[dx] = ((9 * ph * IW + lrow + dx) * 64 + kq * 16) ^ (((((lrow + dx) >> 2) ^ ph) & 1) << 5);
  int L[2];
#pragma unroll
  for (int e = 0; e < 2; ++e) {
    int ry, rx;
    a_pix(ph, 9 + e, lrow, ry, rx);
    L[e] = ((ry * IW + rx) * 64 + kq * 16) ^ ((ry & 1) << 5);
  }
  mma_run<9, APT>(acc, rin, wl, pre, [&](int ks, int j) {
    const int dy = ks / 3, dx = ks % 3;
    if (j < 9) return (A0[dx] + (j + dy) * IW * 64) ^ (((j + dy) & 1) << 5);
    return (L[j - 9] + (dy * IW + dx) * 64) ^ ((dy & 1) << 5);
  });
}

template <bool X2>
__device__ __forceinline__ void epi_a(const PairArgs& a, TileXY t, bool inner, const f32x4 (&acc)[2][APT],
                                      unsigned char* rh, const float4 (&sbp)[2], const float4 (&tbp)[2], int cp, int ph,
                                      int lrow, int kq) {
#pragma unroll
  for (int ct = 0; ct < 2; ++ct) {
    const int cc = (2 * cp + ct) * 16 + kq * 4;
    const float4 s = sbp[ct], sh = tbp[ct];
    const int c8 = (2 * cp + ct) * 2 + (kq >> 1);
    u32x2 xv[X2 ? APT : 1];
    if constexpr (X2) {
#pragma unroll
      for (int j = 0; j < APT; ++j) {
        int ry, rx;
        a_pix(ph, j, lrow, ry, rx);
        const int gy = min(max(t.ty0 - 1 + ry, 0), a.H - 1), gx = min(max(t.tx0 - 1 + rx, 0), a.W - 1);
        xv[j] = *reinterpret_cast<const u32x2*>(a.x2 + (((size_t)t.n * a.H + gy) * a.W + gx) * 64 + cc);
      }
    }
#pragma unroll
    for (int j = 0; j < APT; ++j) {
      int ry, rx;
      if (!a_pix(ph, j, lrow, ry, rx)) continue;
      const int off = (ry * RW + rx) * 128 + ((c8 ^ (((rx >> 1) & 3) << 1)) << 4) + (kq & 1) * 8;
      const int gy = t.ty0 - 1 + ry, gx = t.tx0 - 1 + rx;
      u32x2 st = (u32x2){0u, 0u};
      if (inner || (gy >= 0 && gy < a.H && gx >= 0 && gx < a.W)) {
        float v0 = acc[ct][j][0], v1 = acc[ct][j][1], v2 = acc[ct][j][2], v3 = acc[ct][j][3];
        if constexpr (X2) {
          v0 += lo_bf(xv[j][0]); v1 += hi_bf(xv[j][0]); v2 += lo_bf(xv[j][1]); v3 += hi_bf(xv[j][1]);
        }
        st[0] = relu_bf16x2(pack2bf(fmaf(v0, s.x, sh.x), fmaf(v1, s.y, sh.y)));
        st[1] = relu_bf16x2(pack2bf(fmaf(v2, s.z, sh.z), fmaf(v3, s.w, sh.w)));
      }
      *reinterpret_cast<u32x2*>(rh + off) = st;
    }
  }
}

__device__ __forceinline__ void mma_b(f32x4 (&acc)[2][BPT], const unsigned char* rh, const bf16_t* wl, const WPre& pre,
                                      int ph, int lrow, int kq) {
  int B0[3];
#pragma unroll
  for (int dx = 0; dx < 3; ++dx)
    B0[dx] = (8 * ph * RW + lrow + dx) * 128 + ((kq ^ ((((lrow + dx) >> 1) & 3) << 1)) << 4);
  mma_run<18, BPT>(acc, rh, wl, pre, [&](int s, int pt) {
    const int cb = s / 9, ks = s % 9, dy = ks / 3, dx = ks % 3;
    return (B0[dx] + (pt + dy) * RW * 128) ^ (cb << 6);
  });
}

struct Res {
  u32x2 rv[BPT][2];
  float4 bias[2];
};

template <int RES>
__device__ __forceinline__ void issue_res(const PairArgs& a, TileXY t, int cp, int ph, int lrow, int kq, Res& r) {
#pragma unroll
  for (int pt = 0; pt < BPT; ++pt) {
    const int py = min(t.ty0 + 8 * ph + pt, a.H - 1), px = min(t.tx0 + lrow, a.W - 1);
    const bf16_t* rp = RES == 1 ? a.res + (((size_t)t.n * a.H + py) * a.W + px) * 64 + cp * 32 + kq * 4
                                : a.res + (((size_t)t.n * (a.H >> 1) + (py >> 1)) * (a.W >> 1) + (px >> 1)) * 64 + cp * 32 + kq * 4;
#pragma unroll
    for (int ct = 0; ct < 2; ++ct) r.rv[pt][ct] = *reinterpret_cast<const u32x2*>(rp + ct * 16);
  }
#pragma unroll
  for (int ct = 0; ct < 2; ++ct) r.bias[ct] = *reinterpret_cast<const float4*>(a.bias + (2 * cp + ct) * 16 + kq * 4);
}

struct ProjW {
  bf16x8 w[2];
  float4 b[2];
};

__device__ __forceinline__ void issue_projw(const PairArgs& a, int cp, int lane, ProjW& p) {
#pragma unroll
  for (int ct = 0; ct < 2; ++ct) {
    p.w[ct] = *reinterpret_cast<const bf16x8*>(a.wpf + (2 * cp + ct) * 512 + lane * 8);
    p.b[ct] = *reinterpret_cast<const float4*>(a.biasp + (2 * cp + ct) * 16 + (lane >> 4) * 4);
  }
}

__device__ __forceinline__ void proj_res(const PairArgs& a, const unsigned char* preg, const ProjW& p, int cp, int ph,
                                         int lrow, int kq, Res& r) {
  const f32x4 zero = {0.f, 0.f, 0.f, 0.f};
  const int P0 = ((8 * ph * TS + lrow) * 64 + kq * 16) ^ (((lrow >> 2) & 1) << 5);
#pragma unroll
  for (int pt = 0; pt < BPT; ++pt) {
    const bf16x8 b = *reinterpret_cast<const bf16x8*>(preg + ((P0 + pt * TS * 64) ^ ((pt & 1) << 5)));
#pragma unroll
    for (int ct = 0; ct < 2; ++ct) {
      const f32x4 v = __builtin_amdgcn_mfma_f32_16x16x32_bf16(p.w[ct], b, zero, 0, 0, 0);
      r.rv[pt][ct][0] = pack2bf(v[0] + p.b[ct].x + 0.0f, v[1] + p.b[ct].y + 0.0f);
      r.rv[pt][ct][1] = pack2bf(v[2] + p.b[ct].z + 0.0f, v[3] + p.b[ct].w + 0.0f);
    }
  }
#pragma unroll
  for (int ct = 0; ct < 2; ++ct) r.bias[ct] = *reinterpret_cast<const float4*>(a.bias + (2 * cp + ct) * 16 + kq * 4);
}

__device__ __forceinline__ void epi_b(const PairArgs& a, TileXY t, const f32x4 (&acc)[2][BPT], const Res& r,
                                      unsigned char* ws, int cp, int ph, int lrow, int kq, bool act) {
  const __amdgpu_buffer_rsrc_t rs = __builtin_amdgcn_make_buffer_rsrc(
      a.out + (size_t)t.n * a.H * a.W * 64, (short)0, a.H * a.W * 128, 0x00020000);
#pragma unroll
  for (int ct = 0; ct < 2; ++ct) {
    const float4 bias = r.bias[ct];
    const int ow = lrow * 64 + ((((2 * ct) | (kq >> 1)) ^ ((lrow >> 1) & 3)) << 4) + (kq & 1) * 8;
#pragma unroll
    for (int pt = 0; pt < BPT; ++pt) {
      u32x2 rv = r.rv[pt][ct];
      asm volatile("" : "+v"(rv));
      u32x2 st;
      st[0] = pack2bf(acc[ct][pt][0] + bias.x + lo_bf(rv[0]), acc[ct][pt][1] + bias.y + hi_bf(rv[0]));
      st[1] = pack2bf(acc[ct][pt][2] + bias.z + lo_bf(rv[1]), acc[ct][pt][3] + bias.w + hi_bf(rv[1]));
      *reinterpret_cast<u32x2*>(ws + ow + pt * 1024) = st;
    }
  }
  __builtin_amdgcn_fence(__ATOMIC_RELEASE, "wavefront");
  __builtin_amdgcn_wave_barrier();
  __builtin_amdgcn_fence(__ATOMIC_ACQUIRE, "wavefront");
  const int lane = lrow + 16 * kq;
  const int rd = (lane >> 2) * 64 + (((lane & 3) ^ ((lane >> 3) & 3)) << 4);
  const int px = t.tx0 + (lane >> 2);
#pragma unroll
  for (int it = 0; it < BPT; ++it) {
    const int py = t.ty0 + 8 * ph + it;
    const u32x4 v = *reinterpret_cast<const u32x4*>(ws + rd + it * 1024);
    const int off = (act && py < a.H && px < a.W) ? ((py * a.W + px) * 64 + cp * 32 + (lane & 3) * 8) * 2 : 0x7ffffff0;
    __builtin_amdgcn_raw_buffer_store_b128(v, rs, off, 0, 0);
  }
}

template <int NCA, int INMODE, bool X2, int RES, bool STAMP = false, bool PROJ = false>
__global__ __launch_bounds__(NTP, 2) void conv_pair_pp64_kernel(PairArgs a) {
  static_assert(PROJ ? (NCA == 1 && RES == 0 && !X2) : RES != 0, "the residual is read or projected");
  constexpr int CIN = 32 * NCA;
  unsigned long long ph_work[7] = {0, 0, 0, 0, 0, 0, 0}, ph_wait[7] = {0, 0, 0, 0, 0, 0, 0};
  unsigned long long tstamp = STAMP ? __builtin_amdgcn_s_memtime() : 0;
  auto pre = [&](int i) {
    if constexpr (STAMP) {
      const unsigned long long tn = __builtin_amdgcn_s_memtime();
      ph_work[i] += tn - tstamp;
      tstamp = tn;
    }
  };
  auto post = [&](int i) {
    if constexpr (STAMP) {
      const unsigned long long tn = __builtin_amdgcn_s_memtime();
      ph_wait[i] += tn - tstamp;
      tstamp = tn;
    }
  };
  auto slot = [](int c) { return c > 0 ? 2 : 0; };
  extern __shared__ __attribute__((aligned(16))) unsigned char smem[];
  const int tid0 = threadIdx.x;
  const int total = a.N * a.tiles_x * a.tiles_y;
  const int t0 = (int)(((long long)blockIdx.x * total) / gridDim.x);
  const int t1 = (int)(((long long)(blockIdx.x + 1) * total) / gridDim.x);
  if (t0 >= t1) return;
  const int grp = __builtin_amdgcn_readfirstlane(tid0 / GT);
  const int gt0 = tid0 & (GT - 1);
  unsigned char* reg = smem + grp * RB;
  unsigned char* preg = smem + 2 * RB + grp * P_B;
  Halo<INMODE> halo;
  PAff paff;
  issue_halo<CIN, INMODE>(a, tile16(a, min(t0 + grp, t1 - 1)), 0, gt0, halo);
  if constexpr (PROJ) issue_paff(a, gt0, paff);
  if (grp == 1) __builtin_amdgcn_s_barrier();
  const int iters = (t1 - t0 + 1) >> 1;
  for (int k = 0; k < iters; ++k) {
    int gt = gt0;
    asm volatile("" : "+v"(gt));
    const int gw = __builtin_amdgcn_readfirstlane(gt >> 6), lane = gt & 63, lrow = lane & 15, kq = lane >> 4;
    const int cp = gw & 1, ph = gw >> 1;
    const int t = t0 + 2 * k + grp;
    const bool act = t < t1;
    const TileXY cur = tile16(a, act ? t : t1 - 1);
    const bool inner = interior(a, cur);
    const bf16_t* wla = w_lane(a.waf, cp, lane);
    const bf16_t* wlb = w_lane(a.wbf, cp, lane);
    f32x4 acc_a[2][APT];
#pragma unroll
    for (int i = 0; i < 2; ++i)
#pragma unroll
      for (int j = 0; j < APT; ++j) acc_a[i][j] = (f32x4){0.f, 0.f, 0.f, 0.f};
    WPre wpre;
    float4 sbp[2], tbp[2];
#pragma unroll
    for (int c = 0; c < NCA; ++c) {
      int gc = gt0;
      asm volatile("" : "+v"(gc));
      if constexpr (PROJ)
        commit<INMODE, true>(a, cur, c, gc, inner, halo, reg, &paff, preg);
      else
        commit<INMODE>(a, cur, c, gc, inner, halo, reg);
      issue_w(wla + c * 9 * WSTEP, wpre);
      pre(slot(c));
      __syncthreads();
      post(slot(c));
      if (c + 1 < NCA) issue_halo<CIN, INMODE>(a, cur, c + 1, gt, halo);
      if (c == NCA - 1) {
#pragma unroll
        for (int ct = 0; ct < 2; ++ct) {
          sbp[ct] = *reinterpret_cast<const float4*>(a.sb + (2 * cp + ct) * 16 + kq * 4);
          tbp[ct] = *reinterpret_cast<const float4*>(a.tb + (size_t)cur.n * a.tb_ns + (2 * cp + ct) * 16 + kq * 4);
        }
      }
      __builtin_amdgcn_s_setprio(1);
      mma_a(acc_a, reg, wla + c * 9 * WSTEP, wpre, ph, lrow, kq);
      __builtin_amdgcn_s_setprio(0);
      pre(slot(c) + 1);
      __syncthreads();
      post(slot(c) + 1);
    }
    int g3 = gt0;
    asm volatile("" : "+v"(g3));
    ProjW pw;
    if constexpr (PROJ) issue_projw(a, cp, g3 & 63, pw);
    epi_a<X2>(a, cur, inner, acc_a, reg, sbp, tbp, cp, ph, g3 & 15, (g3 & 63) >> 4);
    Res res;
    if constexpr (PROJ) {
      issue_w(wlb, wpre);
      proj_res(a, preg, pw, cp, ph, g3 & 15, (g3 & 63) >> 4, res);
    } else {
      issue_res<RES>(a, cur, cp, ph, g3 & 15, (g3 & 63) >> 4, res);
      issue_w(wlb, wpre);
    }
    pre(4);
    __syncthreads();
    post(4);
    int g4 = gt0;
    asm volatile("" : "+v"(g4));
    f32x4 acc_b[2][BPT];
#pragma unroll
    for (int i = 0; i < 2; ++i)
#pragma unroll
      for (int j = 0; j < BPT; ++j) acc_b[i][j] = (f32x4){0.f, 0.f, 0.f, 0.f};
    __builtin_amdgcn_s_setprio(1);
    mma_b(acc_b, reg, wlb, wpre, ph, g4 & 15, (g4 & 63) >> 4);
    __builtin_amdgcn_s_setprio(0);
    pre(5);
    __syncthreads();
    post(5);
    int g5 = gt0;
    asm volatile("" : "+v"(g5));
    if constexpr (INMODE != 2) issue_halo<CIN, INMODE>(a, tile16(a, min(t + 2, t1 - 1)), 0, g5, halo);
    __builtin_amdgcn_sched_barrier(0);
    epi_b(a, cur, acc_b, res, reg + gw * OUTW_B, cp, ph, g5 & 15, (g5 & 63) >> 4, act);
    __builtin_amdgcn_sched_barrier(0);
    if constexpr (INMODE == 2) issue_halo<CIN, INMODE>(a, tile16(a, min(t + 2, t1 - 1)), 0, g5, halo);
    if constexpr (PROJ) issue_paff(a, g5, paff);
    pre(6);
    __syncthreads();
    post(6);
  }
  if (grp == 0) __builtin_amdgcn_s_barrier();
  if constexpr (STAMP) {
    if ((tid0 & (GT - 1)) < 16) {
      const int k = tid0 & 15;
      unsigned long long v = 0;
#pragma unroll
      for (int i = 0; i < 7; ++i) {
        if (k == i) v = ph_work[i];
        if (k == 8 + i) v = ph_wait[i];
      }
      if (k == 15) v = (unsigned long long)iters;
      a.stamps[((size_t)blockIdx.x * 2 + grp) * 16 + k] = v;
    }
  }
}
}
```

### csrc/kernels/conv_pp128.hip

```cpp
#include "common.h"

namespace {
namespace pp128 {
constexpr int TH = 8, TW = 28;
constexpr int GW = 4, GT = GW * 64, NTP = 2 * GT;
constexpr int IH = TH + 2, IW = TW + 2, IPIX = IH * IW;
constexpr int IN_B = IPIX * 64;
constexpr int LDS = 2 * IN_B;
constexpr int NF = 14, FC = 7;
constexpr int NCH = 4;
constexpr int C = 128;
constexpr int HU = IPIX * 4, HUPT = (HU + GT - 1) / GT;
constexpr int WD = 3;
constexpr int WSTEP = 8 * 64 * 8;
constexpr int BD = 6, BR = 7;
static_assert(IW % 4 == 2, "the swizzle derivation needs 30 y = 2 y (mod 4)");
constexpr int PJ_B = TH * TW * 128;
constexpr int LDS_PROJ = LDS + 2 * PJ_B;
static_assert(LDS_PROJ <= 128 * 1024, "LDS budget of the ping-pong kernels");
static_assert(BD < BR, "ring");

struct Args {
  const bf16_t* x = nullptr;
  const float* sa = nullptr;
  const float* ta = nullptr;
  const bf16_t* wf = nullptr;
  const float* bias = nullptr;
  const bf16_t* res = nullptr;
  bf16_t* out = nullptr;
  int N = 0, H = 0, W = 0;
  int sa_ns = 0, ta_ns = 0;
  int relu = 0;
  int res_up2 = 0;
  int tiles_x = 0, tiles_y = 0;
  const float* sp = nullptr;
  const float* tp = nullptr;
  const bf16_t* wpf = nullptr;
  const float* bias_p = nullptr;
  bf16_t* out2 = nullptr;
  unsigned long long* stamps = nullptr;
  const float* qs = nullptr;
  const float* qt = nullptr;
  int qrelu = 0;
};

struct TileXY {
  int n, ty0, tx0;
};

__device__ __forceinline__ TileXY tile_of(const Args& a, int t) {
  const int tpi = a.tiles_x * a.tiles_y;
  TileXY r;
  r.n = t / tpi;
  const int q = t - r.n * tpi;
  r.ty0 = (q / a.tiles_x) * TH;
  r.tx0 = (q % a.tiles_x) * TW;
  return r;
}

template <bool POOL>
struct Halo {
  u32x4 h[HUPT];
  float4 aff[4];
};

template <>
struct Halo<true> {
  u32x4 h[HUPT], hb[HUPT];
  u32x4 q[HUPT], qb[HUPT];
  float4 aff[4];
  float4 affp[4];
};

template <bool POOL>
__device__ __forceinline__ void issue_aff(const Args& a, TileXY t, int c, Halo<POOL>& hr) {
  hr.aff[0] = hr.aff[1] = make_float4(1.f, 1.f, 1.f, 1.f);
  hr.aff[2] = hr.aff[3] = make_float4(0.f, 0.f, 0.f, 0.f);
  if (a.sa) {
    const float* sr = a.sa + (size_t)t.n * a.sa_ns + c;
    hr.aff[0] = *reinterpret_cast<const float4*>(sr);
    hr.aff[1] = *reinterpret_cast<const float4*>(sr + 4);
  }
  if (a.ta) {
    const float* tr = a.ta + (size_t)t.n * a.ta_ns + c;
    hr.aff[2] = *reinterpret_cast<const float4*>(tr);
    hr.aff[3] = *reinterpret_cast<const float4*>(tr + 4);
  }
}

__device__ __forceinline__ size_t pool_src(const Args& a, int n, int gy, int gx, int row, int c) {
  return (((size_t)n * 2 * a.H + 2 * gy + row) * 2 * a.W + 2 * gx) * 64 + c;
}

template <bool POOL>
__device__ __forceinline__ void issue_halo(const Args& a, TileXY t, int ch, int gt, Halo<POOL>& hr) {
  const int c = ch * 32 + (gt & 3) * 8;
  if constexpr (!POOL) issue_aff(a, t, c, hr);
#pragma unroll
  for (int i = 0; i < HUPT; ++i) {
    const int pi = min(gt + i * GT, HU - 1) >> 2;
    const int y = pi / IW, x = pi - y * IW;
    const int gy = min(max(t.ty0 - 1 + y, 0), a.H - 1);
    const int gx = min(max(t.tx0 - 1 + x, 0), a.W - 1);
    if constexpr (POOL) {
      const bf16_t* p = a.x + pool_src(a, t.n, gy, gx, 0, c);
      hr.h[i] = *reinterpret_cast<const u32x4*>(p);
      hr.hb[i] = *reinterpret_cast<const u32x4*>(p + 64);
    } else {
      hr.h[i] = *reinterpret_cast<const u32x4*>(a.x + (((size_t)t.n * a.H + gy) * a.W + gx) * C + c);
    }
  }
}

__device__ __forceinline__ void issue_halo_b(const Args& a, TileXY t, int ch, int gt, Halo<true>& hr) {
  const int c = ch * 32 + (gt & 3) * 8;
  issue_aff(a, t, c, hr);
#pragma unroll
  for (int i = 0; i < HUPT; ++i) {
    const int pi = min(gt + i * GT, HU - 1) >> 2;
    const int y = pi / IW, x = pi - y * IW;
    const int gy = min(max(t.ty0 - 1 + y, 0), a.H - 1);
    const int gx = min(max(t.tx0 - 1 + x, 0), a.W - 1);
    const bf16_t* p = a.x + pool_src(a, t.n, gy, gx, 1, c);
    hr.q[i] = *reinterpret_cast<const u32x4*>(p);
    hr.qb[i] = *reinterpret_cast<const u32x4*>(p + 64);
  }
}

__device__ __forceinline__ void issue_affp(const Args& a, int ch, int gt, Halo<true>& hr) {
  const int c = ch * 32 + (gt & 3) * 8;
  hr.affp[0] = *reinterpret_cast<const float4*>(a.sp + c);
  hr.affp[1] = *reinterpret_cast<const float4*>(a.sp + c + 4);
  hr.affp[2] = *reinterpret_cast<const float4*>(a.tp + c);
  hr.affp[3] = *reinterpret_cast<const float4*>(a.tp + c + 4);
}

__device__ __forceinline__ uint32_t max_bf16x2(uint32_t p, uint32_t q) {
  const float lo = fmaxf(lo_bf(p), lo_bf(q)), hi = fmaxf(hi_bf(p), hi_bf(q));
  return (__float_as_uint(lo) >> 16) | (__float_as_uint(hi) & 0xffff0000u);
}

__device__ __forceinline__ void reduce_a(Halo<true>& hr) {
#pragma unroll
  for (int i = 0; i < HUPT; ++i)
#pragma unroll
    for (int j = 0; j < 4; ++j) hr.h[i][j] = max_bf16x2(hr.h[i][j], hr.hb[i][j]);
}

__device__ __forceinline__ void reduce_b(Halo<true>& hr) {
#pragma unroll
  for (int i = 0; i < HUPT; ++i)
#pragma unroll
    for (int j = 0; j < 4; ++j) hr.h[i][j] = max_bf16x2(hr.h[i][j], max_bf16x2(hr.q[i][j], hr.qb[i][j]));
}

template <bool POOL>
__device__ __forceinline__ void commit(const Args& a, TileXY t, int gt, const Halo<POOL>& hr, unsigned char* rin) {
  const int c = gt & 3;
  const float sc[8] = {hr.aff[0].x, hr.aff[0].y, hr.aff[0].z, hr.aff[0].w, hr.aff[1].x, hr.aff[1].y, hr.aff[1].z, hr.aff[1].w};
  const float sh[8] = {hr.aff[2].x, hr.aff[2].y, hr.aff[2].z, hr.aff[2].w, hr.aff[3].x, hr.aff[3].y, hr.aff[3].z, hr.aff[3].w};
  const bool relu = a.relu != 0;
#pragma unroll
  for (int i = 0; i < HUPT; ++i) {
    const int u = gt + i * GT;
    if (u >= HU) continue;
    const int pi = u >> 2;
    const int y = pi / IW, x = pi - y * IW;
    const int gy = t.ty0 - 1 + y, gx = t.tx0 - 1 + x;
    u32x4 pk = (u32x4){0u, 0u, 0u, 0u};
    if (gy >= 0 && gy < a.H && gx >= 0 && gx < a.W) {
#pragma unroll
      for (int j = 0; j < 4; ++j) {
        const float lo = lo_bf(hr.h[i][j]), hi = hi_bf(hr.h[i][j]);
        pk[j] = pack2bf(fmaf(lo, sc[2 * j], sh[2 * j]), fmaf(hi, sc[2 * j + 1], sh[2 * j + 1]));
        if (relu) pk[j] = relu_bf16x2(pk[j]);
      }
    }
    *reinterpret_cast<u32x4*>(rin + pi * 64 + ((c ^ (((x >> 1) & 1) << 1)) << 4)) = pk;
  }
}

__device__ __forceinline__ void commit_proj(int ch, int gt, const Halo<true>& hr, unsigned char* rpj) {
  const int c = gt & 3;
  const float sc[8] = {hr.affp[0].x, hr.affp[0].y, hr.affp[0].z, hr.affp[0].w, hr.affp[1].x, hr.affp[1].y, hr.affp[1].z, hr.affp[1].w};
  const float sh[8] = {hr.affp[2].x, hr.affp[2].y, hr.affp[2].z, hr.affp[2].w, hr.affp[3].x, hr.affp[3].y, hr.affp[3].z, hr.affp[3].w};
#pragma unroll
  for (int i = 0; i < HUPT; ++i) {
    const int u = gt + i * GT;
    if (u >= HU) continue;
    const int pi = u >> 2;
    const int y = pi / IW, x = pi - y * IW;
    if (y < 1 || y > TH || x < 1 || x > TW) continue;
    const int py = y - 1, px = x - 1;
    u32x4 pj;
#pragma unroll
    for (int j = 0; j < 4; ++j)
      pj[j] = pack2bf(fmaf(lo_bf(hr.h[i][j]), sc[2 * j], sh[2 * j]), fmaf(hi_bf(hr.h[i][j]), sc[2 * j + 1], sh[2 * j + 1]));
    *reinterpret_cast<u32x4*>(rpj + (py * TW + px) * 128 + (((ch * 4 + c) ^ (((px >> 1) & 1) << 1) ^ ((py & 1) << 2)) << 4)) = pj;
  }
}

struct WPre {
  bf16x8 w[WD][2];
};

__device__ __forceinline__ const bf16_t* w_lane(const bf16_t* wf, int cp, int lane) {
  return wf + cp * 2 * 512 + lane * 8;
}

__device__ __forceinline__ void issue_w(const bf16_t* wl, WPre& p) {
#pragma unroll
  for (int d = 0; d < WD; ++d)
#pragma unroll
    for (int ct = 0; ct < 2; ++ct) p.w[d][ct] = *reinterpret_cast<const bf16x8*>(wl + d * WSTEP + ct * 512);
}

__device__ __forceinline__ void mma_chunk(f32x4 (&acc)[2][NF], const unsigned char* rin, const bf16_t* wl, const WPre& pre,
                                          const int (&A0)[3]) {
  bf16x8 w[9][2];
#pragma unroll
  for (int d = 0; d < WD; ++d) {
    w[d][0] = pre.w[d][0];
    w[d][1] = pre.w[d][1];
  }
  auto rd = [&](int f) {
    const int s = f / NF, j = f % NF, dy = s / 3, dx = s % 3;
    return *reinterpret_cast<const bf16x8*>(rin + A0[dx] + ((4 * (j / FC) + dy) * IW + 4 * (j % FC)) * 64);
  };
  bf16x8 bf[BR];
#pragma unroll
  for (int f = 0; f < BD; ++f) bf[f] = rd(f);
#pragma unroll
  for (int s = 0; s < 9; ++s) {
    if (s + WD < 9) {
#pragma unroll
      for (int ct = 0; ct < 2; ++ct)
        w[s + WD][ct] = *reinterpret_cast<const bf16x8*>(wl + (s + WD) * WSTEP + ct * 512);
    }
    __builtin_amdgcn_sched_barrier(0);
#pragma unroll
    for (int j = 0; j < NF; ++j) {
      const int f = s * NF + j;
      if (f + BD < 9 * NF) bf[(f + BD) % BR] = rd(f + BD);
#pragma unroll
      for (int ct = 0; ct < 2; ++ct)
        acc[ct][j] = __builtin_amdgcn_mfma_f32_16x16x32_bf16(w[s][ct], bf[f % BR], acc[ct][j], 0, 0, 0);
      __builtin_amdgcn_sched_barrier(0);
    }
  }
}

__device__ __forceinline__ void proj_mma(f32x4 (&acc)[2][NF], const unsigned char* rpj, const bf16_t* wl, int lrow, int kq) {
  bf16x8 w[2][2];
#pragma unroll
  for (int s = 0; s < 2; ++s)
#pragma unroll
    for (int ct = 0; ct < 2; ++ct) w[s][ct] = *reinterpret_cast<const bf16x8*>(wl + s * WSTEP + ct * 512);
  const int ly = lrow >> 2, lx = lrow & 3;
  const int P0 = (ly * TW + lx) * 128 + ((kq ^ (((lx >> 1) & 1) << 1) ^ ((ly & 1) << 2)) << 4);
#pragma unroll
  for (int i = 0; i < 2; ++i)
#pragma unroll
    for (int j = 0; j < NF; ++j) acc[i][j] = (f32x4){0.f, 0.f, 0.f, 0.f};
  auto rd = [&](int f) {
    const int s = f / NF, j = f % NF;
    return *reinterpret_cast<const bf16x8*>(rpj + (P0 ^ (s << 6)) + (4 * (j / FC) * TW + 4 * (j % FC)) * 128);
  };
  constexpr int PD = 3, PR = 4;
  bf16x8 bf[PR];
#pragma unroll
  for (int f = 0; f < PD; ++f) bf[f] = rd(f);
  __builtin_amdgcn_sched_barrier(0);
#pragma unroll
  for (int f = 0; f < 2 * NF; ++f) {
    if (f + PD < 2 * NF) bf[(f + PD) % PR] = rd(f + PD);
#pragma unroll
    for (int ct = 0; ct < 2; ++ct)
      acc[ct][f % NF] = __builtin_amdgcn_mfma_f32_16x16x32_bf16(w[f / NF][ct], bf[f % PR], acc[ct][f % NF], 0, 0, 0);
    __builtin_amdgcn_sched_barrier(0);
  }
}

template <int RES, bool FULL>
__device__ __forceinline__ void epilogue(const Args& a, TileXY t, const f32x4 (&acc)[2][NF], int cp, int lrow, int kq,
                                         bool act) {
  const int ly = lrow >> 2, lx = lrow & 3;
  const int co = cp * 32 + kq * 4;
  const int img_b = a.H * a.W * C * 2;
  const size_t img = (size_t)t.n * a.H * a.W * C;
  const int Wr = a.W >> 1;
  const __amdgpu_buffer_rsrc_t rr = __builtin_amdgcn_make_buffer_rsrc(
      const_cast<bf16_t*>(RES == 2 ? a.res + (size_t)t.n * (a.H >> 1) * Wr * C : (RES ? a.res + img : a.x)), (short)0,
      RES == 2 ? (a.H >> 1) * Wr * C * 2 : (RES ? img_b : 0), 0x00020000);
  const __amdgpu_buffer_rsrc_t ro = __builtin_amdgcn_make_buffer_rsrc(a.out + img, (short)0, img_b, 0x00020000);
  const __amdgpu_buffer_rsrc_t rb = __builtin_amdgcn_make_buffer_rsrc(
      const_cast<float*>(a.bias ? a.bias : a.sa), (short)0, a.bias ? C * 4 : 0, 0x00020000);
  auto voff = [&](int j, int y, int x) {
    if constexpr (FULL) return (((t.ty0 + y) * a.W + t.tx0 + x) * C + co) * 2;
    const int py = t.ty0 + 4 * (j / FC) + y, px = t.tx0 + 4 * (j % FC) + x;
    return (py < a.H && px < a.W) ? ((py * a.W + px) * C + co) * 2 : 0x7ffffff0;
  };
  auto soff = [&](int j) { return FULL ? ((j / FC) * 4 * a.W + (j % FC) * 4) * C * 2 : 0; };
  auto voff_r = [&](int j, int y, int x) {
    if constexpr (FULL) return ((((t.ty0 + y) >> 1) * Wr + ((t.tx0 + x) >> 1)) * C + co) * 2;
    const int py = t.ty0 + 4 * (j / FC) + y, px = t.tx0 + 4 * (j % FC) + x;
    return (py < a.H && px < a.W) ? (((py >> 1) * Wr + (px >> 1)) * C + co) * 2 : 0x7ffffff0;
  };
  auto soff_r = [&](int j) { return FULL ? ((j / FC) * 2 * Wr + (j % FC) * 2) * C * 2 : 0; };
  u32x2 rv[RES ? NF : 1][2];
  f32x4 bias[2];
#pragma unroll
  for (int ct = 0; ct < 2; ++ct)
    bias[ct] = __builtin_bit_cast(f32x4, __builtin_amdgcn_raw_buffer_load_b128(rb, (co + ct * 16) * 4, 0, 0));
  if constexpr (RES != 0) {
#pragma unroll
    for (int j = 0; j < NF; ++j) {
      const int o = RES == 2 ? voff_r(j, ly, lx) : voff(j, ly, lx);
      const int so = RES == 2 ? soff_r(j) : soff(j);
#pragma unroll
      for (int ct = 0; ct < 2; ++ct) rv[j][ct] = __builtin_amdgcn_raw_buffer_load_b64(rr, o + ct * 32, so, 0);
    }
  } else {
#pragma unroll
    for (int ct = 0; ct < 2; ++ct) bias[ct] = bias[ct] + (f32x4){0.f, 0.f, 0.f, 0.f};
  }
  __builtin_amdgcn_sched_barrier(0);
  int sy = ly, sx = lx;
  asm volatile("" : "+v"(sy), "+v"(sx));
#pragma unroll
  for (int j = 0; j < NF; ++j) {
    const int o = act ? voff(j, sy, sx) : 0x7ffffff0;
#pragma unroll
    for (int ct = 0; ct < 2; ++ct) {
      u32x2 st;
      if constexpr (RES != 0) {
        const u32x2 r = rv[j][ct];
        st[0] = pack2bf(acc[ct][j][0] + bias[ct][0] + lo_bf(r[0]), acc[ct][j][1] + bias[ct][1] + hi_bf(r[0]));
        st[1] = pack2bf(acc[ct][j][2] + bias[ct][2] + lo_bf(r[1]), acc[ct][j][3] + bias[ct][3] + hi_bf(r[1]));
      } else {
        st[0] = pack2bf(acc[ct][j][0] + bias[ct][0], acc[ct][j][1] + bias[ct][1]);
        st[1] = pack2bf(acc[ct][j][2] + bias[ct][2], acc[ct][j][3] + bias[ct][3]);
      }
      __builtin_amdgcn_raw_buffer_store_b64(st, ro, o + ct * 32, soff(j), 0);
    }
  }
}

template <bool FULL>
__device__ __forceinline__ void epilogue_c256(const Args& a, TileXY t, int half, const f32x4 (&acc)[2][NF], int cp, int lrow,
                                              int kq, bool act) {
  constexpr int CO = 2 * C;
  const int ly = lrow >> 2, lx = lrow & 3;
  const int co = half * C + cp * 32 + kq * 4;
  const int img_b = a.H * a.W * CO * 2;
  const __amdgpu_buffer_rsrc_t ro =
      __builtin_amdgcn_make_buffer_rsrc(a.out + (size_t)t.n * a.H * a.W * CO, (short)0, img_b, 0x00020000);
  const __amdgpu_buffer_rsrc_t rb = __builtin_amdgcn_make_buffer_rsrc(
      const_cast<float*>(a.bias ? a.bias : a.qs), (short)0, a.bias ? CO * 4 : 0, 0x00020000);
  const __amdgpu_buffer_rsrc_t rs = __builtin_amdgcn_make_buffer_rsrc(const_cast<float*>(a.qs), (short)0, CO * 4, 0x00020000);
  const __amdgpu_buffer_rsrc_t rt = __builtin_amdgcn_make_buffer_rsrc(const_cast<float*>(a.qt), (short)0, CO * 4, 0x00020000);
  auto voff = [&](int j, int y, int x) {
    if constexpr (FULL) return (((t.ty0 + y) * a.W + t.tx0 + x) * CO + co) * 2;
    const int py = t.ty0 + 4 * (j / FC) + y, px = t.tx0 + 4 * (j % FC) + x;
    return (py < a.H && px < a.W) ? ((py * a.W + px) * CO + co) * 2 : 0x7ffffff0;
  };
  auto soff = [&](int j) { return FULL ? ((j / FC) * 4 * a.W + (j % FC) * 4) * CO * 2 : 0; };
  f32x4 bias[2], qs[2], qt[2];
#pragma unroll
  for (int ct = 0; ct < 2; ++ct) {
    bias[ct] = __builtin_bit_cast(f32x4, __builtin_amdgcn_raw_buffer_load_b128(rb, (co + ct * 16) * 4, 0, 0));
    qs[ct] = __builtin_bit_cast(f32x4, __builtin_amdgcn_raw_buffer_load_b128(rs, (co + ct * 16) * 4, 0, 0));
    qt[ct] = __builtin_bit_cast(f32x4, __builtin_amdgcn_raw_buffer_load_b128(rt, (co + ct * 16) * 4, 0, 0));
    bias[ct] = bias[ct] + (f32x4){0.f, 0.f, 0.f, 0.f};
  }
  const bool qrelu = a.qrelu != 0;
  __builtin_amdgcn_sched_barrier(0);
#pragma unroll
  for (int j = 0; j < NF; ++j) {
    const int o = act ? voff(j, ly, lx) : 0x7ffffff0;
#pragma unroll
    for (int ct = 0; ct < 2; ++ct) {
      const uint32_t p0 = pack2bf(acc[ct][j][0] + bias[ct][0], acc[ct][j][1] + bias[ct][1]);
      const uint32_t p1 = pack2bf(acc[ct][j][2] + bias[ct][2], acc[ct][j][3] + bias[ct][3]);
      u32x2 st;
      st[0] = pack2bf(fmaf(lo_bf(p0), qs[ct][0], qt[ct][0]), fmaf(hi_bf(p0), qs[ct][1], qt[ct][1]));
      st[1] = pack2bf(fmaf(lo_bf(p1), qs[ct][2], qt[ct][2]), fmaf(hi_bf(p1), qs[ct][3], qt[ct][3]));
      if (qrelu) {
        st[0] = relu_bf16x2(st[0]);
        st[1] = relu_bf16x2(st[1]);
      }
      __builtin_amdgcn_raw_buffer_store_b64(st, ro, o + ct * 32, soff(j), 0);
    }
  }
}

template <bool STAMP = false, bool POOL = false, bool PROJ = false, bool C256 = false>
__global__ __launch_bounds__(NTP, 2) void conv_pp128_kernel(Args a) {
  static_assert(POOL || !PROJ, "the projection reads the pooled input");
  static_assert(!(POOL && C256), "the 256-channel build reads a plain 128-channel input");
  constexpr int NC = POOL ? 2 : NCH;
  unsigned long long ph_work[5] = {0, 0, 0, 0, 0}, ph_wait[5] = {0, 0, 0, 0, 0};
  unsigned long long tstamp = STAMP ? __builtin_amdgcn_s_memtime() : 0;
  auto pre = [&](int i) {
    if constexpr (STAMP) {
      const unsigned long long tn = __builtin_amdgcn_s_memtime();
      ph_work[i] += tn - tstamp;
      tstamp = tn;
    }
  };
  auto post = [&](int i) {
    if constexpr (STAMP) {
      const unsigned long long tn = __builtin_amdgcn_s_memtime();
      ph_wait[i] += tn - tstamp;
      tstamp = tn;
    }
  };
  auto slot = [](int c) { return c > 0 ? 2 : 0; };
  extern __shared__ __attribute__((aligned(16))) unsigned char smem[];
  const int tid0 = threadIdx.x;
  const int total = a.N * a.tiles_x * a.tiles_y * (C256 ? 2 : 1);
  auto tile_at = [&](int item) { return tile_of(a, C256 ? item >> 1 : item); };
  const int t0 = (int)(((long long)blockIdx.x * total) / gridDim.x);
  const int t1 = (int)(((long long)(blockIdx.x + 1) * total) / gridDim.x);
  if (t0 >= t1) return;
  const int grp = __builtin_amdgcn_readfirstlane(tid0 / GT);
  const int gt0 = tid0 & (GT - 1);
  unsigned char* reg = smem + grp * IN_B;
  unsigned char* rpj = PROJ ? smem + LDS + grp * PJ_B : nullptr;
  Halo<POOL> halo;
  issue_halo(a, tile_at(min(t0 + grp, t1 - 1)), 0, gt0, halo);
  if constexpr (POOL) issue_halo_b(a, tile_at(min(t0 + grp, t1 - 1)), 0, gt0, halo);
  if constexpr (PROJ) issue_affp(a, 0, gt0, halo);
  if (grp == 1) __builtin_amdgcn_s_barrier();
  const int iters = (t1 - t0 + 1) >> 1;
  for (int k = 0; k < iters; ++k) {
    int gt = gt0;
    asm volatile("" : "+v"(gt));
    const int cp = __builtin_amdgcn_readfirstlane(gt >> 6), lane = gt & 63, lrow = lane & 15, kq = lane >> 4;
    const int t = t0 + 2 * k + grp;
    const bool act = t < t1;
    const TileXY cur = tile_at(act ? t : t1 - 1);
    const bf16_t* wl = w_lane(C256 ? a.wf + ((act ? t : t1 - 1) & 1) * (NCH * 9 * WSTEP) : a.wf, cp, lane);
    int A0[3];
#pragma unroll
    for (int dx = 0; dx < 3; ++dx) {
      const int x = (lrow & 3) + dx;
      A0[dx] = ((lrow >> 2) * IW + x) * 64 + ((kq ^ (((x >> 1) & 1) << 1)) << 4);
    }
    f32x4 acc[2][NF];
#pragma unroll
    for (int i = 0; i < 2; ++i)
#pragma unroll
      for (int j = 0; j < NF; ++j) acc[i][j] = (f32x4){0.f, 0.f, 0.f, 0.f};
    WPre wpre;
#pragma unroll
    for (int c = 0; c < NC; ++c) {
      int gc = gt0;
      asm volatile("" : "+v"(gc));
      if constexpr (POOL) {
        reduce_a(halo);
        if (c > 0) {
          __builtin_amdgcn_sched_barrier(0);
          issue_halo_b(a, cur, c, gc, halo);
        }
        reduce_b(halo);
        if constexpr (PROJ) {
          if (c > 0) {
            __builtin_amdgcn_sched_barrier(0);
            issue_affp(a, c, gc, halo);
          }
        }
      }
      commit(a, cur, gc, halo, reg);
      if constexpr (PROJ) {
        __builtin_amdgcn_sched_barrier(0);
        commit_proj(c, gc, halo, rpj);
      }
      __builtin_amdgcn_sched_barrier(0);
      if (c + 1 < NC)
        issue_halo(a, cur, c + 1, gc, halo);
      else
        issue_halo(a, tile_at(min(t + 2, t1 - 1)), 0, gc, halo);
      issue_w(wl + c * 9 * WSTEP, wpre);
      pre(slot(c));
      __syncthreads();
      post(slot(c));
      __builtin_amdgcn_s_setprio(1);
      mma_chunk(acc, reg, wl + c * 9 * WSTEP, wpre, A0);
      __builtin_amdgcn_s_setprio(0);
      pre(slot(c) + 1);
      __syncthreads();
      post(slot(c) + 1);
    }
    int g3 = gt0;
    asm volatile("" : "+v"(g3));
    const bool full = cur.ty0 + TH <= a.H && cur.tx0 + TW <= a.W;
    if constexpr (POOL) {
      if constexpr (!PROJ) {
        issue_halo_b(a, tile_at(min(t + 2, t1 - 1)), 0, g3, halo);
        __builtin_amdgcn_sched_barrier(0);
      }
      if (full)
        epilogue<0, true>(a, cur, acc, cp, g3 & 15, (g3 & 63) >> 4, act);
      else
        epilogue<0, false>(a, cur, acc, cp, g3 & 15, (g3 & 63) >> 4, act);
      if constexpr (PROJ) {
        __builtin_amdgcn_sched_barrier(0);
        int g4 = gt0;
        asm volatile("" : "+v"(g4));
        proj_mma(acc, rpj, w_lane(a.wpf, cp, g4 & 63), g4 & 15, (g4 & 63) >> 4);
        Args b = a;
        b.out = a.out2;
        b.bias = a.bias_p;
        if (full)
          epilogue<0, true>(b, cur, acc, cp, g4 & 15, (g4 & 63) >> 4, act);
        else
          epilogue<0, false>(b, cur, acc, cp, g4 & 15, (g4 & 63) >> 4, act);
        __builtin_amdgcn_sched_barrier(0);
        issue_halo_b(a, tile_at(min(t + 2, t1 - 1)), 0, g4, halo);
        issue_affp(a, 0, g4, halo);
      }
    } else if constexpr (C256) {
      const int half = (act ? t : t1 - 1) & 1;
      if (full)
        epilogue_c256<true>(a, cur, half, acc, cp, g3 & 15, (g3 & 63) >> 4, act);
      else
        epilogue_c256<false>(a, cur, half, acc, cp, g3 & 15, (g3 & 63) >> 4, act);
    } else if (a.res != nullptr && a.res_up2) {
      if (full)
        epilogue<2, true>(a, cur, acc, cp, g3 & 15, (g3 & 63) >> 4, act);
      else
        epilogue<2, false>(a, cur, acc, cp, g3 & 15, (g3 & 63) >> 4, act);
    } else if (a.res != nullptr) {
      if (full)
        epilogue<1, true>(a, cur, acc, cp, g3 & 15, (g3 & 63) >> 4, act);
      else
        epilogue<1, false>(a, cur, acc, cp, g3 & 15, (g3 & 63) >> 4, act);
    } else {
      if (full)
        epilogue<0, true>(a, cur, acc, cp, g3 & 15, (g3 & 63) >> 4, act);
      else
        epilogue<0, false>(a, cur, acc, cp, g3 & 15, (g3 & 63) >> 4, act);
    }
    pre(4);
    __syncthreads();
    post(4);
  }
  if (grp == 0) __builtin_amdgcn_s_barrier();
  if constexpr (STAMP) {
    if ((tid0 & (GT - 1)) < 16) {
      const int k = tid0 & 15;
      unsigned long long v = 0;
#pragma unroll
      for (int i = 0; i < 5; ++i) {
        if (k == i) v = ph_work[i];
        if (k == 8 + i) v = ph_wait[i];
      }
      if (k == 15) v = (unsigned long long)iters;
      a.stamps[((size_t)blockIdx.x * 2 + grp) * 16 + k] = v;
    }
  }
}
}

int g_pp128 = be_env_int("BE_CONV_PP128", 1);

int g_pp128_res_up2 = be_env_int("BE_CONV_PP128_RES_UP2", 1);

int g_pp128_pool = be_env_int("BE_CONV_PP128_POOL", 1);

int g_pp128_pool_proj = be_env_int("BE_CONV_PP128_POOL_PROJ", 1);

int g_l3_prepool = be_env_int("BE_CPNET_L3_PREPOOL", 1);

int g_pp128_c256 = be_env_int("BE_CONV_PP128_C256", 1);

int g_pp128_c256_launches = 0;
int g_pp128_grid = 0;
int g_pp128_launches = 0;
int g_pp128_pool_launches = 0;
unsigned long long* g_pp128_stamps = nullptr;
int g_pp128_stamps_cap = 0;

int pp128_grid_for(int N, int H, int W, int* tiles_x, int* tiles_y, int halves = 1) {
  if (!g_pp128 || N <= 0 || H <= 0 || W <= 0 || (long long)H * W * 256 * halves >= (1LL << 31) - 64) return 0;
  const int tx = (W + pp128::TW - 1) / pp128::TW, ty = (H + pp128::TH - 1) / pp128::TH;
  const long long tiles = (long long)N * tx * ty * halves;
  const bool forced = g_pp128_grid > 0;
  const int g = forced ? (int)(tiles < g_pp128_grid ? tiles : g_pp128_grid) : 256;
  if (!(forced || tiles >= 2LL * g) || tiles >= (1LL << 30)) return 0;
  if (tiles_x) *tiles_x = tx;
  if (tiles_y) *tiles_y = ty;
  return g;
}

pp128::Args pp128_args(const void* x, const float* pscale, const float* pshift, int pshift_ns, int pscale_ns, int prelu,
                       const void* wfrag, const float* bias, void* out, int N, int H, int W) {
  pp128::Args a;
  a.x = (const bf16_t*)x; a.sa = pscale; a.ta = pshift; a.sa_ns = pscale_ns; a.ta_ns = pshift_ns;
  a.wf = (const bf16_t*)wfrag; a.bias = bias; a.out = (bf16_t*)out;
  a.N = N; a.H = H; a.W = W; a.relu = prelu & 1;
  a.stamps = g_pp128_stamps;
  return a;
}

template <bool POOL, bool PROJ, bool C256>
int pp128_launch(const pp128::Args& a, int grid, hipStream_t stream) {
  constexpr int lds = PROJ ? pp128::LDS_PROJ : pp128::LDS;
  if constexpr (PROJ) {
    static bool attr_set[BE_MAX_DEV] = {};
    if (!attr_set[be_cur_dev()]) {
      if (hipFuncSetAttribute(reinterpret_cast<const void*>(&pp128::conv_pp128_kernel<false, POOL, PROJ, C256>),
                              hipFuncAttributeMaxDynamicSharedMemorySize, lds) != hipSuccess ||
          hipFuncSetAttribute(reinterpret_cast<const void*>(&pp128::conv_pp128_kernel<true, POOL, PROJ, C256>),
                              hipFuncAttributeMaxDynamicSharedMemorySize, lds) != hipSuccess)
        return -33;
      attr_set[be_cur_dev()] = true;
    }
  }
  if (a.stamps != nullptr) {
    if (grid > g_pp128_stamps_cap) return -30;
    hipLaunchKernelGGL((pp128::conv_pp128_kernel<true, POOL, PROJ, C256>), dim3(grid), dim3(pp128::NTP), lds, stream, a);
  } else {
    hipLaunchKernelGGL((pp128::conv_pp128_kernel<false, POOL, PROJ, C256>), dim3(grid), dim3(pp128::NTP), lds, stream, a);
  }
  return BE_CHECK_LAUNCH();
}

}

extern "C" {

int be_conv2d_nhwc(const void* x, const void* x2, const float* pscale, const float* pshift, int pshift_ns, int pscale_ns,
                   int prelu, const void* w, const float* bias, const void* res, void* out, int N, int H, int W,
                   int Hs, int Ws, int Cin, int Cout, int cout_valid, int ks, int ck, int tco, int inmode,
                   int out_f32_nchw, int nw, const float* qscale, const float* qshift, int qshift_ns,
                   hipStream_t stream);

int be_conv_pp128_set_grid(int blocks) {
  g_pp128_grid = blocks;
  return 0;
}

int be_conv_pp128_set_stamps(void* buf, int cap_workgroups) {
  g_pp128_stamps = static_cast<unsigned long long*>(buf);
  g_pp128_stamps_cap = buf ? cap_workgroups : 0;
  return 0;
}

int be_conv_pp128_launches() { return g_pp128_launches; }

int be_conv2d_nhwc_frag_res(const void* x, const void* x2, const float* pscale, const float* pshift, int pshift_ns,
                            int pscale_ns, int prelu, const void* w, const float* bias, const void* res, void* out,
                            int N, int H, int W, int Hs, int Ws, int Cin, int Cout, int cout_valid, int ks, int ck,
                            int tco, int inmode, int out_f32_nchw, int nw, const float* qscale, const float* qshift,
                            int qshift_ns, const void* wfrag, int res_up2, hipStream_t stream) {
  const bool frag_ok = wfrag && ks == 3 && ck == 32 && !x2 && !out_f32_nchw && Cout == 128 && !(prelu & 2) && !qscale &&
                       !qshift && x && out;
  const bool shape_ok = frag_ok && inmode == 0 && Cin == 128 && Hs == H && Ws == W;
  if (res_up2 && !(shape_ok && res && H % 2 == 0 && W % 2 == 0)) return -31;
  const bool pool_ok = frag_ok && g_pp128_pool && inmode == 2 && Cin == 64 && Hs == 2 * H && Ws == 2 * W && !res;
  if (shape_ok || pool_ok) {
    pp128::Args a = pp128_args(x, pscale, pshift, pshift_ns, pscale_ns, prelu, wfrag, bias, out, N, H, W);
    const int g = pp128_grid_for(N, H, W, &a.tiles_x, &a.tiles_y);
    if (g > 0 && pool_ok) {
      ++g_pp128_pool_launches;
      return pp128_launch<true, false, false>(a, g, stream);
    }
    if (g > 0) {
      a.res = (const bf16_t*)res;
      a.res_up2 = res_up2 ? 1 : 0;
      ++g_pp128_launches;
      return pp128_launch<false, false, false>(a, g, stream);
    }
  }
  if (res_up2) return -31;
  return be_conv2d_nhwc(x, x2, pscale, pshift, pshift_ns, pscale_ns, prelu, w, bias, res, out, N, H, W, Hs, Ws, Cin, Cout,
                        cout_valid, ks, ck, tco, inmode, out_f32_nchw, nw, qscale, qshift, qshift_ns, stream);
}

int be_conv2d_nhwc_frag(const void* x, const void* x2, const float* pscale, const float* pshift, int pshift_ns,
                        int pscale_ns, int prelu, const void* w, const float* bias, const void* res, void* out, int N,
                        int H, int W, int Hs, int Ws, int Cin, int Cout, int cout_valid, int ks, int ck, int tco,
                        int inmode, int out_f32_nchw, int nw, const float* qscale, const float* qshift, int qshift_ns,
                        const void* wfrag, hipStream_t stream) {
  return be_conv2d_nhwc_frag_res(x, x2, pscale, pshift, pshift_ns, pscale_ns, prelu, w, bias, res, out, N, H, W, Hs, Ws,
                                 Cin, Cout, cout_valid, ks, ck, tco, inmode, out_f32_nchw, nw, qscale, qshift,
                                 qshift_ns, wfrag, 0, stream);
}

int be_conv_pp128_takes(int N, int H, int W) { return pp128_grid_for(N, H, W, nullptr, nullptr) > 0 ? 1 : 0; }

int be_conv_pp128_takes_pool(int N, int Hs, int Ws) {
  return g_pp128_pool && Hs % 2 == 0 && Ws % 2 == 0 && pp128_grid_for(N, Hs / 2, Ws / 2, nullptr, nullptr) > 0 ? 1 : 0;
}

int be_conv_pp128_set_pool(int pool, int pool_proj) {
  g_pp128_pool = pool;
  g_pp128_pool_proj = pool_proj;
  return 0;
}

int be_conv_pp128_pool_launches() { return g_pp128_pool_launches; }

int be_conv_pp128_takes_pool_proj(int N, int Hs, int Ws) {
  return g_pp128_pool_proj && be_conv_pp128_takes_pool(N, Hs, Ws);
}

int be_conv_pp128_pool_proj(const void* x, const float* pscale, const float* pshift, int pshift_ns, int pscale_ns, int prelu,
                            const void* wfrag, const float* bias, void* out, const float* sp, const float* tp,
                            const void* wpfrag, const float* bias_p, void* out2, int N, int Hs, int Ws,
                            hipStream_t stream) {
  if (!x || !wfrag || !out || !sp || !tp || !wpfrag || !out2 || out == out2 || (prelu & ~1)) return -32;
  if (!be_conv_pp128_takes_pool_proj(N, Hs, Ws)) return -32;
  pp128::Args a = pp128_args(x, pscale, pshift, pshift_ns, pscale_ns, prelu, wfrag, bias, out, N, Hs / 2, Ws / 2);
  const int g = pp128_grid_for(N, Hs / 2, Ws / 2, &a.tiles_x, &a.tiles_y);
  a.sp = sp; a.tp = tp; a.wpf = (const bf16_t*)wpfrag; a.bias_p = bias_p; a.out2 = (bf16_t*)out2;
  ++g_pp128_pool_launches;
  return pp128_launch<true, true, false>(a, g, stream);
}

static int pp128_c256_grid_for(int N, int H, int W, int* tiles_x, int* tiles_y) {
  return pp128_grid_for(N, H, W, tiles_x, tiles_y, 2);
}

int be_conv_pp128_takes_prepool(int N, int H, int W) {
  return g_l3_prepool && pp128_c256_grid_for(N, H, W, nullptr, nullptr) > 0 ? 1 : 0;
}

int be_conv_pp128_takes_c256(int N, int H, int W) { return g_pp128_c256 && be_conv_pp128_takes_prepool(N, H, W); }

int be_conv_pp128_set_c256(int prepool, int c256) {
  g_l3_prepool = prepool;
  g_pp128_c256 = c256;
  return 0;
}

int be_conv_pp128_c256_launches() { return g_pp128_c256_launches; }

int be_conv_pp128_c256(const void* x, const float* pscale, const float* pshift, int pshift_ns, int pscale_ns, int prelu,
                       const void* wfrag, const float* bias, void* out, const float* qscale, const float* qshift, int N,
                       int H, int W, hipStream_t stream) {
  if (!x || !wfrag || !out || x == out || !qscale || !qshift || (prelu & ~3)) return -34;
  if (!be_conv_pp128_takes_c256(N, H, W)) return -34;
  pp128::Args a = pp128_args(x, pscale, pshift, pshift_ns, pscale_ns, prelu, wfrag, bias, out, N, H, W);
  const int g = pp128_c256_grid_for(N, H, W, &a.tiles_x, &a.tiles_y);
  a.qs = qscale; a.qt = qshift; a.qrelu = (prelu >> 1) & 1;
  ++g_pp128_c256_launches;
  return pp128_launch<false, false, true>(a, g, stream);
}

int be_conv_pp128_takes_res_up2(int N, int H, int W) {
  return g_pp128_res_up2 && H % 2 == 0 && W % 2 == 0 && be_conv_pp128_takes(N, H, W);
}

}
```

Measured before the change: 2542 img/s.

## Add dynamic atomic tile scheduling to ping-pong conv kernels

Replaces the static contiguous tile range per workgroup in the level0, pp64 and pp128 ping-pong conv kernels with a dynamic work queue. Workgroups fetch the next tile pair from a per-stream global atomic counter and prefetch it into an LDS ring. The last workgroup to finish resets the counters. The aim is to even out load imbalance and tail effects across CUs. It adds atomics, extra template instantiations and host-side stream lookup under a mutex, and it is disabled during graph capture. It applies only when there are at least four iterations per block.

```diff
diff --git a/bioengine_worker_amd/ops/conv_pair.py b/bioengine_worker_amd/ops/conv_pair.py
--- a/bioengine_worker_amd/ops/conv_pair.py
+++ b/bioengine_worker_amd/ops/conv_pair.py
@@ -294,3 +294,32 @@
         _native.ptr(head.b), _native.ptr(hout), head.nh, N, H, W, _native.stream(x.device),
     )
     return hout
+
+
+PP_LEVEL0, PP_PP64, PP_PP128 = 1, 2, 4
+PP_ALL = PP_LEVEL0 | PP_PP64 | PP_PP128
+_native.register_hip_signatures({
+    "be_pp_set_dynamic": "i", "be_pp_get_dynamic": "", "be_pp_dynamic_launches": "", "be_pp_debug_pair": "sp",
+})
+
+
+def pp_dynamic() -> int:
+    return int(_native.hip().be_pp_get_dynamic())
+
+
+def pp_set_dynamic(mask: int) -> None:
+    _native.call("be_pp_set_dynamic", int(mask))
+
+
+def pp_dynamic_launches() -> int:
+    return int(_native.hip().be_pp_dynamic_launches())
+
+
+def pp_debug_pair(stream: torch.cuda.Stream):
+    import ctypes
+
+    words = (ctypes.c_uint32 * 2)()
+    idx = int(_native.hip().be_pp_debug_pair(ctypes.c_void_p(stream.cuda_stream), ctypes.cast(words, ctypes.c_void_p)))
+    if idx < -1:
+        raise RuntimeError(f"be_pp_debug_pair failed with status {idx}")
+    return idx, (int(words[0]), int(words[1]))
diff --git a/csrc/kernels/common.h b/csrc/kernels/common.h
--- a/csrc/kernels/common.h
+++ b/csrc/kernels/common.h
@@ -3,6 +3,7 @@
 #include <stdint.h>
 #include <cstdio>
 #include <cstdlib>
+#include <mutex>
 
 typedef uint16_t bf16_t;
 typedef __attribute__((ext_vector_type(8))) short bf16x8;
@@ -74,3 +75,145 @@
   }
   return z;
 }
+
+#define BE_PP_RING 4
+
+template <bool DYN>
+__device__ __forceinline__ int* be_pp_ring() {
+  if constexpr (DYN) {
+    __shared__ int ring[BE_PP_RING];
+    return ring;
+  } else {
+    return nullptr;
+  }
+}
+
+#define BE_PP_CHUNK_L0 1
+#define BE_PP_CHUNK_PP64 1
+#define BE_PP_CHUNK_PP128 1
+
+template <bool DYN, int CH = 1>
+struct PPTiles {
+  int base, lim;
+  int iters = 0;
+  unsigned int* ctr = nullptr;
+  int* ring = nullptr;
+  int left = CH - 1, seq = 0;
+  unsigned int pend = 0;
+
+  __device__ __forceinline__ int item_of(unsigned int chunk) const {
+    const long long i = (long long)chunk * (2 * CH);
+    return i < lim ? (int)i : lim;
+  }
+  __device__ __forceinline__ unsigned int request() const {
+    return gridDim.x + __hip_atomic_fetch_add(ctr, 1u, __ATOMIC_RELAXED, __HIP_MEMORY_SCOPE_AGENT);
+  }
+  __device__ __forceinline__ bool init(unsigned int* counters, int total, int* ring_words) {
+    if constexpr (DYN) {
+      ctr = counters; ring = ring_words; lim = total;
+      base = item_of(blockIdx.x);
+      if (base >= lim) {
+        finish();
+        return false;
+      }
+      if (threadIdx.x == 0) pend = request();
+      return true;
+    } else {
+      base = (int)(((long long)blockIdx.x * total) / gridDim.x);
+      lim = (int)(((long long)(blockIdx.x + 1) * total) / gridDim.x);
+      return base < lim;
+    }
+  }
+  __device__ __forceinline__ void start() {
+    if constexpr (DYN) {
+      if (threadIdx.x == 0) ring[1] = item_of(pend);
+    }
+  }
+  __device__ __forceinline__ void top() {
+    ++iters;
+    if constexpr (DYN) {
+      if (first() && threadIdx.x == 0) pend = request();
+    }
+  }
+  __device__ __forceinline__ void land() {
+    if constexpr (DYN) {
+      if (first() && threadIdx.x == 0) ring[(seq + 2) & (BE_PP_RING - 1)] = item_of(pend);
+    }
+  }
+  __device__ __forceinline__ bool first() const { return CH == 1 || left == CH - 1; }
+  __device__ __forceinline__ int next() const {
+    if constexpr (DYN) {
+      if (CH == 1 || left == 0) return max(__builtin_amdgcn_readfirstlane(ring[(seq + 1) & (BE_PP_RING - 1)]), 0);
+    }
+    return base + 2;
+  }
+  __device__ __forceinline__ void advance(int next_base) {
+    if constexpr (DYN) {
+      if (CH == 1 || left == 0) {
+        left = CH - 1;
+        ++seq;
+      } else {
+        --left;
+      }
+    }
+    base = next_base;
+  }
+  __device__ __forceinline__ void finish() const {
+    if constexpr (DYN) {
+      if (threadIdx.x == 0) {
+        const unsigned int done = __hip_atomic_fetch_add(ctr + 1, 1u, __ATOMIC_RELAXED, __HIP_MEMORY_SCOPE_AGENT);
+        if (done == gridDim.x - 1) {
+          __hip_atomic_store(ctr, 0u, __ATOMIC_RELAXED, __HIP_MEMORY_SCOPE_AGENT);
+          __hip_atomic_store(ctr + 1, 0u, __ATOMIC_RELAXED, __HIP_MEMORY_SCOPE_AGENT);
+        }
+      }
+    }
+  }
+};
+
+#define BE_PP_LEVEL0 1
+#define BE_PP_PP64 2
+#define BE_PP_PP128 4
+#define BE_PP_PAIRS 64
+#define BE_PP_PAIR_STRIDE 64
+inline int g_pp_dynamic = be_env_int("BE_PP_DYNAMIC", 7);
+inline int g_pp_dynamic_launches = 0;
+
+struct BePPPool {
+  unsigned int* words[BE_MAX_DEV] = {};
+  hipStream_t streams[BE_MAX_DEV][BE_PP_PAIRS] = {};
+  int used[BE_MAX_DEV] = {};
+};
+inline BePPPool g_pp_pool;
+
+inline int be_pp_pair_index(hipStream_t stream, bool create) {
+  static std::mutex mu;
+  std::lock_guard<std::mutex> lock(mu);
+  const int d = be_cur_dev();
+  for (int i = 0; i < g_pp_pool.used[d]; ++i)
+    if (g_pp_pool.streams[d][i] == stream) return i;
+  if (!create || g_pp_pool.used[d] >= BE_PP_PAIRS) return -1;
+  if (!g_pp_pool.words[d]) {
+    const size_t bytes = (size_t)BE_PP_PAIRS * BE_PP_PAIR_STRIDE * sizeof(unsigned int);
+    if (hipMalloc((void**)&g_pp_pool.words[d], bytes) != hipSuccess) { g_pp_pool.words[d] = nullptr; return -1; }
+    if (hipMemset(g_pp_pool.words[d], 0, bytes) != hipSuccess) return -1;
+  }
+  g_pp_pool.streams[d][g_pp_pool.used[d]] = stream;
+  return g_pp_pool.used[d]++;
+}
+
+#define BE_PP_MIN_ITERS 4
+inline unsigned int* be_pp_counters(int family, hipStream_t stream, long long items, int grid, bool forced) {
+  if (!(g_pp_dynamic & family)) return nullptr;
+  if (!forced && items < 2LL * BE_PP_MIN_ITERS * grid) return nullptr;
+  hipStreamCaptureStatus st = hipStreamCaptureStatusNone;
+  if (hipStreamIsCapturing(stream, &st) != hipSuccess) {
+    (void)hipGetLastError();
+    return nullptr;
+  }
+  if (st != hipStreamCaptureStatusNone) return nullptr;
+  const int i = be_pp_pair_index(stream, true);
+  if (i < 0) return nullptr;
+  ++g_pp_dynamic_launches;
+  return g_pp_pool.words[be_cur_dev()] + (size_t)i * BE_PP_PAIR_STRIDE;
+}
diff --git a/csrc/kernels/conv_pair.hip b/csrc/kernels/conv_pair.hip
--- a/csrc/kernels/conv_pair.hip
+++ b/csrc/kernels/conv_pair.hip
@@ -26,6 +26,7 @@
   int N, H, W, Hs, Ws, Cin;
   int tiles_x, tiles_y;
   unsigned long long* stamps;
+  unsigned int* ctr;
 };
 
 namespace g32 {
@@ -594,7 +595,7 @@
 template <bool STEM> struct PPHaloOf { using T = PPHalo; };
 template <> struct PPHaloOf<true> { using T = PPHalo8; };
 
-template <int NCA, int INMODE, bool X2, int RES, bool HEAD, bool STEM = false, bool STAMP = false>
+template <int NCA, int INMODE, bool X2, int RES, bool HEAD, bool STEM = false, bool STAMP = false, bool DYN = false>
 __global__ __launch_bounds__(ppk::NTP, ppk::GW == 4 ? 2 : 4) void conv_pair_pp_kernel(PairArgs a) {
   static_assert(!STEM || (NCA == 1 && INMODE == 0 && !X2 && RES == 0 && !HEAD), "stem configuration");
   constexpr int CIN = 32 * NCA;
@@ -619,9 +620,8 @@
   extern __shared__ __attribute__((aligned(16))) unsigned char smem[];
   const int tid0 = threadIdx.x;
   const int total = a.N * a.tiles_x * a.tiles_y;
-  const int t0 = (int)(((long long)blockIdx.x * total) / gridDim.x);
-  const int t1 = (int)(((long long)(blockIdx.x + 1) * total) / gridDim.x);
-  if (t0 >= t1) return;
+  PPTiles<DYN, BE_PP_CHUNK_L0> ts;
+  if (!ts.init(a.ctr, total, be_pp_ring<DYN>())) return;
   bf16_t* wl = reinterpret_cast<bf16_t*>(smem + 2 * RB);
   const bf16_t* wb = wl + (STEM ? 32 * pps::WSTRA : NCA * 32 * ppk::WSTR);
   const bf16_t* wp = wb + 32 * ppk::WSTR;
@@ -657,17 +657,17 @@
       else pp_issue_halo<INMODE, CIN>(a, nx, 0, gtv, halo);
     }
   };
-  if constexpr (STEM) pp8_issue_halo<false>(a, tile_xy(a, min(t0 + grp, t1 - 1)), gt0, halo);
-  else pp_issue_halo<INMODE, CIN>(a, tile_xy(a, min(t0 + grp, t1 - 1)), 0, gt0, halo);
+  if constexpr (STEM) pp8_issue_halo<false>(a, tile_xy(a, min(ts.base + grp, ts.lim - 1)), gt0, halo);
+  else pp_issue_halo<INMODE, CIN>(a, tile_xy(a, min(ts.base + grp, ts.lim - 1)), 0, gt0, halo);
   __builtin_amdgcn_s_waitcnt((0x7 << 4) | (0xf << 8));
   __syncthreads();
+  ts.start();
   if (grp == 1) __builtin_amdgcn_s_barrier();
-  const int iters = (t1 - t0 + 1) >> 1;
-  for (int k = 0; k < iters; ++k) {
+  while (ts.base < ts.lim) {
     int gt = gt0;
     asm volatile("" : "+v"(gt));
     const int gw = __builtin_amdgcn_readfirstlane(gt >> 6), lane = gt & 63, lrow = lane & 15, kq = lane >> 4;
-    const int t = t0 + 2 * k + grp;
+    const int t = ts.base + grp, t1 = ts.lim;
     const bool act = t < t1;
     const TileXY cur = tile_xy(a, act ? t : t1 - 1);
     const bool inner = pp_interior(a, cur);
@@ -687,6 +687,7 @@
         if (inner) pp_commit<true>(a, cur, gc, halo, reg);
         else pp_commit<false>(a, cur, gc, halo, reg);
       }
+      if (c == 0) ts.top();
       pre(2 * c);
       __syncthreads();
       post(2 * c);
@@ -722,9 +723,14 @@
     asm volatile("" : "+v"(g3));
     if (inner) pp_epi_a<X2, true>(a, cur, acc_a, reg, sb, tb, sk, gw, g3 & 15, (g3 & 63) >> 4);
     else pp_epi_a<X2, false>(a, cur, acc_a, reg, sb, tb, sk, gw, g3 & 15, (g3 & 63) >> 4);
+    ts.land();
     PPRes res;
     if constexpr (PP_VAR & 1) pp_issue_res<RES>(a, cur, gw, g3 & 15, (g3 & 63) >> 4, res);
-    if constexpr (PP_VAR & 8) issue0(tile_xy(a, min(t + 2, t1 - 1)), g3);
+    int nb = 0;
+    if constexpr (PP_VAR & 8) {
+      nb = ts.next();
+      issue0(tile_xy(a, min(nb + grp, t1 - 1)), g3);
+    }
     pre(2 * NCA);
     __syncthreads();
     post(2 * NCA);
@@ -747,7 +753,8 @@
     int g5 = gt0;
     asm volatile("" : "+v"(g5));
     const int lrow5 = g5 & 15, kq5 = (g5 & 63) >> 4;
-    auto next_halo = [&]() { issue0(tile_xy(a, min(t + 2, t1 - 1)), g5); };
+    if constexpr (!(PP_VAR & 8)) nb = ts.next();
+    auto next_halo = [&]() { issue0(tile_xy(a, min(nb + grp, t1 - 1)), g5); };
     if constexpr (!(PP_VAR & 10)) next_halo();
     __builtin_amdgcn_sched_barrier(0);
     if constexpr (HEAD) pp_epi_head(a, cur, acc_b, res, hr, gw, lrow5, kq5, act);
@@ -756,8 +763,10 @@
     pre(2 * NCA + 2);
     __syncthreads();
     post(2 * NCA + 2);
+    ts.advance(nb);
   }
   if (grp == 0) __builtin_amdgcn_s_barrier();
+  ts.finish();
   if constexpr (STAMP) {
     if ((tid0 & (ppk::GT - 1)) < 16) {
       const int k = tid0 & 15;
@@ -767,7 +776,7 @@
         if (k == i) v = ph_work[i];
         if (k == 8 + i) v = ph_wait[i];
       }
-      if (k == 15) v = (unsigned long long)iters;
+      if (k == 15) v = (unsigned long long)ts.iters;
       a.stamps[((size_t)blockIdx.x * 2 + grp) * 16 + k] = v;
     }
   }
@@ -776,10 +785,22 @@
 unsigned long long* g_pp_stamps = nullptr;
 int g_pp_stamps_cap = 0;
 
+template <int NCA, int INMODE, bool X2, int RES, bool HEAD, bool STEM, bool STAMP, bool DYN>
+int launch_pair_pp_k(const PairArgs& a, int g, hipStream_t s) {
+  constexpr int lds = STEM ? pps::LDS : 2 * ppk::RB + (NCA + 1) * ppk::W_B;
+  static_assert(lds <= 160 * 1024, "ping-pong LDS budget");
+  static bool attr_set[BE_MAX_DEV] = {};
+  if (!attr_set[be_cur_dev()]) {
+    hipFuncSetAttribute(reinterpret_cast<const void*>(&conv_pair_pp_kernel<NCA, INMODE, X2, RES, HEAD, STEM, STAMP, DYN>),
+                        hipFuncAttributeMaxDynamicSharedMemorySize, lds);
+    attr_set[be_cur_dev()] = true;
+  }
+  hipLaunchKernelGGL((conv_pair_pp_kernel<NCA, INMODE, X2, RES, HEAD, STEM, STAMP, DYN>), dim3(g), dim3(ppk::NTP), lds, s, a);
+  return BE_CHECK_LAUNCH();
+}
+
 template <int NCA, int INMODE, bool X2, int RES, bool HEAD, bool STEM = false>
 int launch_pair_pp(PairArgs a, int grid_cap, hipStream_t s) {
-  constexpr int lds = STEM ? pps::LDS : 2 * ppk::RB + (NCA + 1) * ppk::W_B;
-  static_assert(lds <= 160 * 1024, "ping-pong LDS budget");
   a.tiles_x = (a.W + TW - 1) / TW;
   a.tiles_y = (a.H + TH - 1) / TH;
   const int tiles = a.N * a.tiles_x * a.tiles_y;
@@ -787,33 +808,35 @@
   if (g > tiles) g = tiles;
   if (g < 1) return 0;
   a.stamps = nullptr;
-  static bool attr_set[BE_MAX_DEV] = {};
-  if (!attr_set[be_cur_dev()]) {
-    hipFuncSetAttribute(reinterpret_cast<const void*>(&conv_pair_pp_kernel<NCA, INMODE, X2, RES, HEAD, STEM>),
-                        hipFuncAttributeMaxDynamicSharedMemorySize, lds);
-    attr_set[be_cur_dev()] = true;
-  }
   if (g_pp_stamps != nullptr) {
     if (g > g_pp_stamps_cap) return -30;
     a.stamps = g_pp_stamps;
-    static bool attr_st[BE_MAX_DEV] = {};
-    if (!attr_st[be_cur_dev()]) {
-      hipFuncSetAttribute(reinterpret_cast<const void*>(&conv_pair_pp_kernel<NCA, INMODE, X2, RES, HEAD, STEM, true>),
-                          hipFuncAttributeMaxDynamicSharedMemorySize, lds);
-      attr_st[be_cur_dev()] = true;
-    }
-    hipLaunchKernelGGL((conv_pair_pp_kernel<NCA, INMODE, X2, RES, HEAD, STEM, true>), dim3(g), dim3(ppk::NTP), lds, s, a);
-    return BE_CHECK_LAUNCH();
-  }
-  hipLaunchKernelGGL((conv_pair_pp_kernel<NCA, INMODE, X2, RES, HEAD, STEM>), dim3(g), dim3(ppk::NTP), lds, s, a);
+  }
+  a.ctr = be_pp_counters(BE_PP_LEVEL0, s, tiles, g, grid_cap > 0);
+  if (a.stamps != nullptr)
+    return a.ctr ? launch_pair_pp_k<NCA, INMODE, X2, RES, HEAD, STEM, true, true>(a, g, s)
+                 : launch_pair_pp_k<NCA, INMODE, X2, RES, HEAD, STEM, true, false>(a, g, s);
+  return a.ctr ? launch_pair_pp_k<NCA, INMODE, X2, RES, HEAD, STEM, false, true>(a, g, s)
+               : launch_pair_pp_k<NCA, INMODE, X2, RES, HEAD, STEM, false, false>(a, g, s);
+}
+
+#include "conv_pair_pp64.inc"
+
+template <int NCA, int INMODE, bool X2, int RES, bool PROJ, bool STAMP, bool DYN>
+int launch_pair_pp64_k(const PairArgs& a, int g, hipStream_t s) {
+  constexpr int lds = PROJ ? pp64::LDS_PROJ : pp64::LDS;
+  static bool attr_set[BE_MAX_DEV] = {};
+  if (!attr_set[be_cur_dev()]) {
+    (void)hipFuncSetAttribute(reinterpret_cast<const void*>(&pp64::conv_pair_pp64_kernel<NCA, INMODE, X2, RES, STAMP, PROJ, DYN>),
+                              hipFuncAttributeMaxDynamicSharedMemorySize, lds);
+    attr_set[be_cur_dev()] = true;
+  }
+  hipLaunchKernelGGL((pp64::conv_pair_pp64_kernel<NCA, INMODE, X2, RES, STAMP, PROJ, DYN>), dim3(g), dim3(pp64::NTP), lds, s, a);
   return BE_CHECK_LAUNCH();
 }
-
-#include "conv_pair_pp64.inc"
 
 template <int NCA, int INMODE, bool X2, int RES, bool PROJ = false>
 int launch_pair_pp64(PairArgs a, int grid_cap, hipStream_t s) {
-  constexpr int lds = PROJ ? pp64::LDS_PROJ : pp64::LDS;
   a.tiles_x = (a.W + pp64::TS - 1) / pp64::TS;
   a.tiles_y = (a.H + pp64::TS - 1) / pp64::TS;
   const int tiles = a.N * a.tiles_x * a.tiles_y;
@@ -821,22 +844,16 @@
   if (g > tiles) g = tiles;
   if (g < 1) return 0;
   a.stamps = nullptr;
-  static bool attr_set[BE_MAX_DEV] = {};
-  if (!attr_set[be_cur_dev()]) {
-    (void)hipFuncSetAttribute(reinterpret_cast<const void*>(&pp64::conv_pair_pp64_kernel<NCA, INMODE, X2, RES, false, PROJ>),
-                              hipFuncAttributeMaxDynamicSharedMemorySize, lds);
-    (void)hipFuncSetAttribute(reinterpret_cast<const void*>(&pp64::conv_pair_pp64_kernel<NCA, INMODE, X2, RES, true, PROJ>),
-                              hipFuncAttributeMaxDynamicSharedMemorySize, lds);
-    attr_set[be_cur_dev()] = true;
-  }
   if (g_pp_stamps != nullptr) {
     if (g > g_pp_stamps_cap) return -30;
     a.stamps = g_pp_stamps;
-    hipLaunchKernelGGL((pp64::conv_pair_pp64_kernel<NCA, INMODE, X2, RES, true, PROJ>), dim3(g), dim3(pp64::NTP), lds, s, a);
-    return BE_CHECK_LAUNCH();
-  }
-  hipLaunchKernelGGL((pp64::conv_pair_pp64_kernel<NCA, INMODE, X2, RES, false, PROJ>), dim3(g), dim3(pp64::NTP), lds, s, a);
-  return BE_CHECK_LAUNCH();
+  }
+  a.ctr = be_pp_counters(BE_PP_PP64, s, tiles, g, grid_cap > 0);
+  if (a.stamps != nullptr)
+    return a.ctr ? launch_pair_pp64_k<NCA, INMODE, X2, RES, PROJ, true, true>(a, g, s)
+                 : launch_pair_pp64_k<NCA, INMODE, X2, RES, PROJ, true, false>(a, g, s);
+  return a.ctr ? launch_pair_pp64_k<NCA, INMODE, X2, RES, PROJ, false, true>(a, g, s)
+               : launch_pair_pp64_k<NCA, INMODE, X2, RES, PROJ, false, false>(a, g, s);
 }
 }
 
@@ -880,6 +897,23 @@
 int be_conv_pair_set_grid(int blocks) {
   g_pair_grid = blocks;
   return 0;
+}
+
+int be_pp_set_dynamic(int mask) {
+  g_pp_dynamic = mask;
+  return 0;
+}
+
+int be_pp_get_dynamic() { return g_pp_dynamic; }
+
+int be_pp_dynamic_launches() { return g_pp_dynamic_launches; }
+
+int be_pp_debug_pair(hipStream_t stream, void* words2) {
+  const int i = be_pp_pair_index(stream, false);
+  if (i >= 0 && words2 != nullptr &&
+      hipMemcpy(words2, g_pp_pool.words[be_cur_dev()] + (size_t)i * BE_PP_PAIR_STRIDE, 8, hipMemcpyDeviceToHost) != hipSuccess)
+    return -41;
+  return i;
 }
 
 int be_conv_pair_set_stamps(void* buf, int cap_workgroups) {
diff --git a/csrc/kernels/conv_pair_pp64.inc b/csrc/kernels/conv_pair_pp64.inc
--- a/csrc/kernels/conv_pair_pp64.inc
+++ b/csrc/kernels/conv_pair_pp64.inc
@@ -346,7 +346,7 @@
   }
 }
 
-template <int NCA, int INMODE, bool X2, int RES, bool STAMP = false, bool PROJ = false>
+template <int NCA, int INMODE, bool X2, int RES, bool STAMP = false, bool PROJ = false, bool DYN = false>
 __global__ __launch_bounds__(NTP, 2) void conv_pair_pp64_kernel(PairArgs a) {
   static_assert(PROJ ? (NCA == 1 && RES == 0 && !X2) : RES != 0, "the residual is read or projected");
   constexpr int CIN = 32 * NCA;
@@ -370,25 +370,24 @@
   extern __shared__ __attribute__((aligned(16))) unsigned char smem[];
   const int tid0 = threadIdx.x;
   const int total = a.N * a.tiles_x * a.tiles_y;
-  const int t0 = (int)(((long long)blockIdx.x * total) / gridDim.x);
-  const int t1 = (int)(((long long)(blockIdx.x + 1) * total) / gridDim.x);
-  if (t0 >= t1) return;
+  PPTiles<DYN, BE_PP_CHUNK_PP64> ts;
+  if (!ts.init(a.ctr, total, be_pp_ring<DYN>())) return;
   const int grp = __builtin_amdgcn_readfirstlane(tid0 / GT);
   const int gt0 = tid0 & (GT - 1);
   unsigned char* reg = smem + grp * RB;
   unsigned char* preg = smem + 2 * RB + grp * P_B;
   Halo<INMODE> halo;
   PAff paff;
-  issue_halo<CIN, INMODE>(a, tile16(a, min(t0 + grp, t1 - 1)), 0, gt0, halo);
+  issue_halo<CIN, INMODE>(a, tile16(a, min(ts.base + grp, ts.lim - 1)), 0, gt0, halo);
   if constexpr (PROJ) issue_paff(a, gt0, paff);
+  ts.start();
   if (grp == 1) __builtin_amdgcn_s_barrier();
-  const int iters = (t1 - t0 + 1) >> 1;
-  for (int k = 0; k < iters; ++k) {
+  while (ts.base < ts.lim) {
     int gt = gt0;
     asm volatile("" : "+v"(gt));
     const int gw = __builtin_amdgcn_readfirstlane(gt >> 6), lane = gt & 63, lrow = lane & 15, kq = lane >> 4;
     const int cp = gw & 1, ph = gw >> 1;
-    const int t = t0 + 2 * k + grp;
+    const int t = ts.base + grp, t1 = ts.lim;
     const bool act = t < t1;
     const TileXY cur = tile16(a, act ? t : t1 - 1);
     const bool inner = interior(a, cur);
@@ -409,6 +408,7 @@
         commit<INMODE, true>(a, cur, c, gc, inner, halo, reg, &paff, preg);
       else
         commit<INMODE>(a, cur, c, gc, inner, halo, reg);
+      if (c == 0) ts.top();
       issue_w(wla + c * 9 * WSTEP, wpre);
       pre(slot(c));
       __syncthreads();
@@ -433,6 +433,7 @@
     ProjW pw;
     if constexpr (PROJ) issue_projw(a, cp, g3 & 63, pw);
     epi_a<X2>(a, cur, inner, acc_a, reg, sbp, tbp, cp, ph, g3 & 15, (g3 & 63) >> 4);
+    ts.land();
     Res res;
     if constexpr (PROJ) {
       issue_w(wlb, wpre);
@@ -459,17 +460,20 @@
     post(5);
     int g5 = gt0;
     asm volatile("" : "+v"(g5));
-    if constexpr (INMODE != 2) issue_halo<CIN, INMODE>(a, tile16(a, min(t + 2, t1 - 1)), 0, g5, halo);
+    const int nb = ts.next();
+    if constexpr (INMODE != 2) issue_halo<CIN, INMODE>(a, tile16(a, min(nb + grp, t1 - 1)), 0, g5, halo);
     __builtin_amdgcn_sched_barrier(0);
     epi_b(a, cur, acc_b, res, reg + gw * OUTW_B, cp, ph, g5 & 15, (g5 & 63) >> 4, act);
     __builtin_amdgcn_sched_barrier(0);
-    if constexpr (INMODE == 2) issue_halo<CIN, INMODE>(a, tile16(a, min(t + 2, t1 - 1)), 0, g5, halo);
+    if constexpr (INMODE == 2) issue_halo<CIN, INMODE>(a, tile16(a, min(nb + grp, t1 - 1)), 0, g5, halo);
     if constexpr (PROJ) issue_paff(a, g5, paff);
     pre(6);
     __syncthreads();
     post(6);
+    ts.advance(nb);
   }
   if (grp == 0) __builtin_amdgcn_s_barrier();
+  ts.finish();
   if constexpr (STAMP) {
     if ((tid0 & (GT - 1)) < 16) {
       const int k = tid0 & 15;
@@ -479,7 +483,7 @@
         if (k == i) v = ph_work[i];
         if (k == 8 + i) v = ph_wait[i];
       }
-      if (k == 15) v = (unsigned long long)iters;
+      if (k == 15) v = (unsigned long long)ts.iters;
       a.stamps[((size_t)blockIdx.x * 2 + grp) * 16 + k] = v;
     }
   }
diff --git a/csrc/kernels/conv_pp128.hip b/csrc/kernels/conv_pp128.hip
--- a/csrc/kernels/conv_pp128.hip
+++ b/csrc/kernels/conv_pp128.hip
@@ -42,6 +42,7 @@
   const float* qs = nullptr;
   const float* qt = nullptr;
   int qrelu = 0;
+  unsigned int* ctr = nullptr;
 };
 
 struct TileXY {
@@ -394,7 +395,7 @@
   }
 }
 
-template <bool STAMP = false, bool POOL = false, bool PROJ = false, bool C256 = false>
+template <bool STAMP = false, bool POOL = false, bool PROJ = false, bool C256 = false, bool DYN = false>
 __global__ __launch_bounds__(NTP, 2) void conv_pp128_kernel(Args a) {
   static_assert(POOL || !PROJ, "the projection reads the pooled input");
   static_assert(!(POOL && C256), "the 256-channel build reads a plain 128-channel input");
@@ -420,24 +421,24 @@
   const int tid0 = threadIdx.x;
   const int total = a.N * a.tiles_x * a.tiles_y * (C256 ? 2 : 1);
   auto tile_at = [&](int item) { return tile_of(a, C256 ? item >> 1 : item); };
-  const int t0 = (int)(((long long)blockIdx.x * total) / gridDim.x);
-  const int t1 = (int)(((long long)(blockIdx.x + 1) * total) / gridDim.x);
-  if (t0 >= t1) return;
+  PPTiles<DYN, BE_PP_CHUNK_PP128> ts;
+  if (!ts.init(a.ctr, total, be_pp_ring<DYN>())) return;
   const int grp = __builtin_amdgcn_readfirstlane(tid0 / GT);
   const int gt0 = tid0 & (GT - 1);
   unsigned char* reg = smem + grp * IN_B;
   unsigned char* rpj = PROJ ? smem + LDS + grp * PJ_B : nullptr;
   Halo<POOL> halo;
-  issue_halo(a, tile_at(min(t0 + grp, t1 - 1)), 0, gt0, halo);
-  if constexpr (POOL) issue_halo_b(a, tile_at(min(t0 + grp, t1 - 1)), 0, gt0, halo);
+  issue_halo(a, tile_at(min(ts.base + grp, ts.lim - 1)), 0, gt0, halo);
+  if constexpr (POOL) issue_halo_b(a, tile_at(min(ts.base + grp, ts.lim - 1)), 0, gt0, halo);
   if constexpr (PROJ) issue_affp(a, 0, gt0, halo);
+  ts.start();
   if (grp == 1) __builtin_amdgcn_s_barrier();
-  const int iters = (t1 - t0 + 1) >> 1;
-  for (int k = 0; k < iters; ++k) {
+  while (ts.base < ts.lim) {
     int gt = gt0;
     asm volatile("" : "+v"(gt));
     const int cp = __builtin_amdgcn_readfirstlane(gt >> 6), lane = gt & 63, lrow = lane & 15, kq = lane >> 4;
-    const int t = t0 + 2 * k + grp;
+    const int t = ts.base + grp, t1 = ts.lim;
+    int nb = 0;
     const bool act = t < t1;
     const TileXY cur = tile_at(act ? t : t1 - 1);
     const bf16_t* wl = w_lane(C256 ? a.wf + ((act ? t : t1 - 1) & 1) * (NCH * 9 * WSTEP) : a.wf, cp, lane);
@@ -477,10 +478,14 @@
         commit_proj(c, gc, halo, rpj);
       }
       __builtin_amdgcn_sched_barrier(0);
-      if (c + 1 < NC)
+      if (c == 0) ts.top();
+      if (c == 1) ts.land();
+      if (c + 1 < NC) {
         issue_halo(a, cur, c + 1, gc, halo);
-      else
-        issue_halo(a, tile_at(min(t + 2, t1 - 1)), 0, gc, halo);
+      } else {
+        nb = ts.next();
+        issue_halo(a, tile_at(min(nb + grp, t1 - 1)), 0, gc, halo);
+      }
       issue_w(wl + c * 9 * WSTEP, wpre);
       pre(slot(c));
       __syncthreads();
@@ -497,7 +502,7 @@
     const bool full = cur.ty0 + TH <= a.H && cur.tx0 + TW <= a.W;
     if constexpr (POOL) {
       if constexpr (!PROJ) {
-        issue_halo_b(a, tile_at(min(t + 2, t1 - 1)), 0, g3, halo);
+        issue_halo_b(a, tile_at(min(nb + grp, t1 - 1)), 0, g3, halo);
         __builtin_amdgcn_sched_barrier(0);
       }
       if (full)
@@ -517,7 +522,7 @@
         else
           epilogue<0, false>(b, cur, acc, cp, g4 & 15, (g4 & 63) >> 4, act);
         __builtin_amdgcn_sched_barrier(0);
-        issue_halo_b(a, tile_at(min(t + 2, t1 - 1)), 0, g4, halo);
+        issue_halo_b(a, tile_at(min(nb + grp, t1 - 1)), 0, g4, halo);
         issue_affp(a, 0, g4, halo);
       }
     } else if constexpr (C256) {
@@ -545,8 +550,10 @@
     pre(4);
     __syncthreads();
     post(4);
+    ts.advance(nb);
   }
   if (grp == 0) __builtin_amdgcn_s_barrier();
+  ts.finish();
   if constexpr (STAMP) {
     if ((tid0 & (GT - 1)) < 16) {
       const int k = tid0 & 15;
@@ -556,7 +563,7 @@
         if (k == i) v = ph_work[i];
         if (k == 8 + i) v = ph_wait[i];
       }
-      if (k == 15) v = (unsigned long long)iters;
+      if (k == 15) v = (unsigned long long)ts.iters;
       a.stamps[((size_t)blockIdx.x * 2 + grp) * 16 + k] = v;
     }
   }
@@ -604,27 +611,32 @@
   return a;
 }
 
-template <bool POOL, bool PROJ, bool C256>
-int pp128_launch(const pp128::Args& a, int grid, hipStream_t stream) {
+template <bool STAMP, bool POOL, bool PROJ, bool C256, bool DYN>
+int pp128_launch_k(const pp128::Args& a, int grid, hipStream_t stream) {
   constexpr int lds = PROJ ? pp128::LDS_PROJ : pp128::LDS;
   if constexpr (PROJ) {
     static bool attr_set[BE_MAX_DEV] = {};
     if (!attr_set[be_cur_dev()]) {
-      if (hipFuncSetAttribute(reinterpret_cast<const void*>(&pp128::conv_pp128_kernel<false, POOL, PROJ, C256>),
-                              hipFuncAttributeMaxDynamicSharedMemorySize, lds) != hipSuccess ||
-          hipFuncSetAttribute(reinterpret_cast<const void*>(&pp128::conv_pp128_kernel<true, POOL, PROJ, C256>),
+      if (hipFuncSetAttribute(reinterpret_cast<const void*>(&pp128::conv_pp128_kernel<STAMP, POOL, PROJ, C256, DYN>),
                               hipFuncAttributeMaxDynamicSharedMemorySize, lds) != hipSuccess)
         return -33;
       attr_set[be_cur_dev()] = true;
     }
   }
-  if (a.stamps != nullptr) {
-    if (grid > g_pp128_stamps_cap) return -30;
-    hipLaunchKernelGGL((pp128::conv_pp128_kernel<true, POOL, PROJ, C256>), dim3(grid), dim3(pp128::NTP), lds, stream, a);
-  } else {
-    hipLaunchKernelGGL((pp128::conv_pp128_kernel<false, POOL, PROJ, C256>), dim3(grid), dim3(pp128::NTP), lds, stream, a);
-  }
+  hipLaunchKernelGGL((pp128::conv_pp128_kernel<STAMP, POOL, PROJ, C256, DYN>), dim3(grid), dim3(pp128::NTP), lds, stream, a);
   return BE_CHECK_LAUNCH();
+}
+
+template <bool POOL, bool PROJ, bool C256>
+int pp128_launch(pp128::Args a, int grid, hipStream_t stream) {
+  if (a.stamps != nullptr && grid > g_pp128_stamps_cap) return -30;
+  const long long items = (long long)a.N * a.tiles_x * a.tiles_y * (C256 ? 2 : 1);
+  a.ctr = be_pp_counters(BE_PP_PP128, stream, items, grid, g_pp128_grid > 0);
+  if (a.stamps != nullptr)
+    return a.ctr ? pp128_launch_k<true, POOL, PROJ, C256, true>(a, grid, stream)
+                 : pp128_launch_k<true, POOL, PROJ, C256, false>(a, grid, stream);
+  return a.ctr ? pp128_launch_k<false, POOL, PROJ, C256, true>(a, grid, stream)
+               : pp128_launch_k<false, POOL, PROJ, C256, false>(a, grid, stream);
 }
 
 }
```

Result: faster. 2574 img/s (median of 5 runs) (+1.2%).
